# alguoo314/JASPER

Measured on AMD Instinct MI355X. Metric: assembly Mbp/s polished + Gk-mers/s counted, k=37, higher is better.
Workload: dtype u64

## Files before the change

jasper_amd/csrc/polish.hip:

```cpp
#include "polish.hpp"
#include <algorithm>

namespace jk {

constexpr int SMAX = 384;

__device__ __forceinline__ void pyslice(int64_t len, int64_t a, int64_t b, int64_t &lo, int64_t &hi) {
    if (a < 0) { a += len; if (a < 0) a = 0; } else if (a > len) a = len;
    if (b < 0) { b += len; if (b < 0) b = 0; } else if (b > len) b = len;
    if (b < a) b = a;
    lo = a; hi = b;
}

__device__ __forceinline__ int64_t pyround(double x) { return (int64_t)rint(x); }

struct FrontEntry {
    uint32_t node;
    uint16_t tlen;
    uint8_t alive;
    uint8_t pad;
    uint8_t tail[72];
};
static_assert(sizeof(FrontEntry) == 80, "FrontEntry layout");

#ifndef JK_POLISH_TICKS
#define JK_POLISH_TICKS 0
#endif
__device__ __forceinline__ uint64_t phase_clock() { return JK_POLISH_TICKS ? wall_clock64() : 0ull; }

struct Walker {
    TableDev T;
    int k, step, lane;
    uint32_t solid;
    uint8_t *buf;
    int64_t len, gs, glen, cap;
    SegDev *C;
    uint32_t chunk_id;
    uint32_t nrec, naux, seqno, nedit;
    int pass;
    int status;
    uint64_t nlook;
    uint64_t tk[12];
    uint8_t *s_tbf, *s_t1, *s_t2, *s_gkb, *s_gka;
    int64_t delta;
    int64_t dirty_end;
    int64_t glo;
    bool is_first, is_last;
    int spec_fail;
    const uint8_t *cls;
    int64_t cls_n, seg_lo, stop_orig;
    ScratchPool pool;
    uint32_t *bfs_nodes;
    uint8_t *bfs_front, *bfs_patch;
    int bfs_slot;

    __device__ __forceinline__ void guard(int64_t lo, int64_t hi) {
        if ((!is_first && lo < glo) || (!is_last && hi > len)) spec_fail = 1;
    }

    __device__ __forceinline__ uint8_t at(int64_t p) const { return buf[p < gs ? p : p + glen]; }

    struct __attribute__((packed, aligned(1))) U16 { uint32_t w[4]; };

    __device__ __forceinline__ void load_window(int64_t lo, int n, uint32_t w[16]) const {
#pragma unroll
        for (int c = 0; c < 4; ++c) {
            const int64_t s = lo + 16 * c;
            U16 v;
            v.w[0] = v.w[1] = v.w[2] = v.w[3] = 0;
            if (16 * c < n) {
                if (s + 16 <= gs) v = *reinterpret_cast<const U16 *>(buf + s);
                else if (s >= gs && s + glen + 16 <= cap) v = *reinterpret_cast<const U16 *>(buf + s + glen);
                else {
#pragma unroll
                    for (int j = 0; j < 16; ++j) {
                        const int64_t p = s + j;
                        const uint32_t b = p < len ? at(p) : 0u;
                        v.w[j >> 2] |= b << (8 * (j & 3));
                    }
                }
            }
#pragma unroll
            for (int j = 0; j < 4; ++j) w[4 * c + j] = v.w[j];
        }
    }
    __device__ __forceinline__ u128 encode_words(const uint32_t w[16], int lim, int &nvalid) const {
        uint64_t hi = 0, lo = 0, inv = 0;
#pragma unroll
        for (int i = 0; i < 16; ++i) {
            const uint32_t x0 = (w[i] >> 1) & 0x03030303u;
            const uint32_t x = x0 ^ ((x0 >> 1) & 0x01010101u);
            const uint32_t expect = __builtin_amdgcn_perm(0u, 0x54474341u, x);
            const uint32_t d = expect ^ (w[i] & 0xDFDFDFDFu);
            const uint32_t nz = (((d & 0x7F7F7F7Fu) + 0x7F7F7F7Fu) | d) & 0x80808080u;
            const uint32_t c8 = (x * 0x40100401u) >> 24;
            const uint32_t n4 = (((nz >> 7) * 0x01020408u) >> 24) & 0xFu;
            if (i < 8) hi |= (uint64_t)c8 << (56 - 8 * i);
            else lo |= (uint64_t)c8 << (56 - 8 * (i - 8));
            inv |= (uint64_t)n4 << (4 * i);
        }
        if (lim < 64) inv |= ~0ull << lim;
        const int t = inv ? (int)__builtin_ctzll(inv) : 64;
        nvalid = t;
        if (t == 0) return mk(0, 0);
        return shl(shr(mk(hi, lo), 128 - 2 * t), 2 * (k - t));
    }

    __device__ __forceinline__ uint32_t cnt_seq(int64_t a, int64_t b) {
        int64_t lo, hi;
        guard(a, b);
        pyslice(len, a, b, lo, hi);
        const int n = (int)(hi - lo < k ? hi - lo : k);
        uint32_t w[16];
        load_window(lo, n, w);
        int nv;
        const u128 m = encode_words(w, n, nv);
        return clamp32(table_get(T, mix(canonical(m, k), T.B)));
    }
    __device__ __forceinline__ uint32_t cnt_str(const uint8_t *p, int n) const {
        const int lim = n < k ? n : k;
        uint32_t w[16];
#pragma unroll
        for (int x = 0; x < 16; ++x) {
            uint32_t v = 0;
#pragma unroll
            for (int y = 0; y < 4; ++y) {
                const int q = 4 * x + y;
                const uint32_t b = q < lim ? (uint32_t)p[q] : 0u;
                v |= b << (8 * y);
            }
            w[x] = v;
        }
        int nv;
        const u128 m = encode_words(w, lim, nv);
        return clamp32(table_get(T, mix(canonical(m, k), T.B)));
    }

    template <typename F>
    __device__ __forceinline__ uint32_t cnt_fn(int n, F get) const {
        const int lim = n < k ? n : k;
        uint32_t w[16];
#pragma unroll
        for (int x = 0; x < 16; ++x) {
            uint32_t v = 0;
#pragma unroll
            for (int y = 0; y < 4; ++y) {
                const int q = 4 * x + y;
                const uint32_t b = q < lim ? (uint32_t)get(q) : 0u;
                v |= b << (8 * y);
            }
            w[x] = v;
        }
        int nv;
        const u128 m = encode_words(w, lim, nv);
        return clamp32(table_get(T, mix(canonical(m, k), T.B)));
    }

    __device__ void move_gap(int64_t to) {
        if (to == gs) return;
        if (to > gs) {
            const int64_t n = to - gs;
            const uint8_t *src = buf + gs + glen;
            uint8_t *dst = buf + gs;
            int64_t off = 0;
            for (; off + 4096 <= n; off += 4096) {
                U16 v[4];
#pragma unroll
                for (int u = 0; u < 4; ++u) v[u] = *reinterpret_cast<const U16 *>(src + off + (u * 64 + lane) * 16);
#pragma unroll
                for (int u = 0; u < 4; ++u) *reinterpret_cast<U16 *>(dst + off + (u * 64 + lane) * 16) = v[u];
            }
            for (; off < n; off += 256) {
                uint8_t v[4];
#pragma unroll
                for (int u = 0; u < 4; ++u) { int64_t q = off + u * 64 + lane; v[u] = q < n ? src[q] : 0; }
#pragma unroll
                for (int u = 0; u < 4; ++u) { int64_t q = off + u * 64 + lane; if (q < n) dst[q] = v[u]; }
            }
        } else {
            const int64_t n = gs - to;
            const uint8_t *src_end = buf + gs;
            uint8_t *dst_end = buf + gs + glen;
            int64_t off = 0;
            for (; off + 4096 <= n; off += 4096) {
                U16 v[4];
#pragma unroll
                for (int u = 0; u < 4; ++u) v[u] = *reinterpret_cast<const U16 *>(src_end - off - (u * 64 + lane + 1) * 16);
#pragma unroll
                for (int u = 0; u < 4; ++u) *reinterpret_cast<U16 *>(dst_end - off - (u * 64 + lane + 1) * 16) = v[u];
            }
            for (; off < n; off += 256) {
                uint8_t v[4];
#pragma unroll
                for (int u = 0; u < 4; ++u) { int64_t q = off + u * 64 + lane; v[u] = q < n ? src_end[-1 - q] : 0; }
#pragma unroll
                for (int u = 0; u < 4; ++u) { int64_t q = off + u * 64 + lane; if (q < n) dst_end[-1 - q] = v[u]; }
            }
        }
        gs = to;
        __builtin_amdgcn_fence(__ATOMIC_SEQ_CST, "workgroup");
    }
    __device__ void replace(int64_t a, int64_t b, const uint8_t *patch, int64_t plen) {
        const uint64_t tr0 = phase_clock();
        replace_(a, b, patch, plen);
        tk[3] += phase_clock() - tr0;
    }
    __device__ void replace_(int64_t a, int64_t b, const uint8_t *patch, int64_t plen) {
        move_gap(a);
        glen += (b - a);
        if (glen < plen) { status = PS_GAP_EXHAUSTED; return; }
        if (nedit >= C->edit_cap) { status = PS_REC_OVERFLOW; return; }
        if (lane == 0) {
            EditRec e;
            e.a = a; e.plen = (int32_t)plen; e.oldlen = (int32_t)(b - a);
            C->edits[nedit] = e;
        }
        nedit++;
        for (int64_t q = lane; q < plen; q += 64) buf[gs + q] = patch[q];
        gs += plen;
        glen -= plen;
        len += plen - (b - a);
        delta += plen - (b - a);
        dirty_end = a + plen;
        __builtin_amdgcn_fence(__ATOMIC_SEQ_CST, "workgroup");
    }

    __device__ __forceinline__ void cp_seq(uint8_t *dst, int64_t lo, int64_t hi) {
        guard(lo, hi);
        for (int64_t q = lane; q < hi - lo; q += 64) dst[q] = at(lo + q);
    }
    __device__ __forceinline__ void cp_mem(uint8_t *dst, const uint8_t *src, int n) const {
        for (int q = lane; q < n; q += 64) dst[q] = src[q];
    }
    __device__ __forceinline__ void put(uint8_t *dst, uint8_t c) const { if (lane == 0) *dst = c; }
    __device__ __forceinline__ void sync() const { __syncthreads(); }

    __device__ bool check_sequence(const uint8_t *t, int n, uint32_t thr) {
        const int nmid = (n - k > step) ? (n - k - step + step - 1) / step : 0;
        const int jobs = 2 + nmid;
        bool ok = true;
        for (int base = 0; base < jobs; base += 64) {
            const int j = base + lane;
            bool bad = false;
            if (j < jobs) {
                uint32_t c;
                if (j == 0) c = cnt_str(t, n < k ? n : k);
                else if (j == 1) { int lo = n > k ? n - k : 0; c = cnt_str(t + lo, n - lo); }
                else { int i = step * (j - 1); c = cnt_str(t + i, k); }
                bad = c < thr;
            }
            if (__ballot(bad)) ok = false;
        }
        nlook += (uint64_t)jobs;
        return ok;
    }
    __device__ int dense_bad(const uint8_t *t, int n, uint32_t thr) {
        int bad = 0;
        const int nw = n - k + 1;
        for (int base = 0; base < nw; base += 64) {
            const int i = base + lane;
            bool b = false;
            if (i < nw) b = cnt_str(t + i, k) < thr;
            bad += __popcll(__ballot(b));
        }
        if (nw > 0) nlook += (uint64_t)nw;
        return bad;
    }

    __device__ void emit(uint8_t kind, int64_t index, uint8_t newc, uint8_t oldc, uint32_t rep, uint32_t aux_off, uint32_t aux_len) {
        if (nrec >= C->rec_cap) { status = PS_REC_OVERFLOW; return; }
        if (lane == 0) {
            FixRec r;
            r.index = index; r.chunk = chunk_id; r.seqno = seqno; r.pass = (uint8_t)pass; r.kind = kind;
            r.newc = newc; r.oldc = oldc; r.rep = rep; r.aux_off = aux_off; r.aux_len = aux_len;
            C->recs[nrec] = r;
        }
        nrec++;
        seqno++;
    }

    __device__ uint8_t fix_k_case_sub(int L, uint32_t thr, int &outlen) {
        const uint8_t bad = s_tbf[k - 1];
        const char *order = "ACTG";
        for (int b = 0; b < 4; ++b) {
            if ((uint8_t)order[b] == bad) continue;
            cp_mem(s_t1, s_tbf, L);
            sync();
            put(s_t1 + k - 1, (uint8_t)order[b]);
            sync();
            if (check_sequence(s_t1, L, thr)) { outlen = L; return (uint8_t)order[b]; }
            sync();
        }
        return 0;
    }
    __device__ uint8_t fix_insert(int L, uint32_t thr, int &outlen) {
        cp_mem(s_t1, s_tbf, k - 1);
        cp_mem(s_t1 + k - 1, s_tbf + k, L - k);
        sync();
        if (check_sequence(s_t1, L - 1, thr)) { outlen = L - 1; return s_tbf[k - 1]; }
        sync();
        return 0;
    }
    __device__ uint8_t fix_del(int L, uint32_t thr, int &outlen) {
        const char *order = "ATCG";
        for (int a = 0; a < 4; ++a) {
            cp_mem(s_t1, s_tbf, k - 1);
            cp_mem(s_t1 + k, s_tbf + k - 1, L - (k - 1));
            put(s_t1 + k - 1, (uint8_t)order[a]);
            sync();
            if (check_sequence(s_t1, L + 1, thr)) { outlen = L + 1; return (uint8_t)order[a]; }
            sync();
        }
        return 0;
    }
    __device__ uint8_t fixdiploid(int L, uint32_t thr, int64_t gb, int64_t ga, uint8_t &left, uint8_t &right, int &outlen) {
        const uint8_t left_bad = s_tbf[L - k], right_bad = s_tbf[k - 1];
        int64_t gbsi = gb - k + 1; if (gbsi < 0) gbsi = 0;
        const int64_t h = (int64_t)((double)(k - 1 - L + k) / 2.0);
        int64_t alo, ahi, blo, bhi;
        if (ga + k - 1 + h < len) pyslice(len, ga + k - 1, ga + k - 1 + h, alo, ahi);
        else {
            if (!is_last) spec_fail = 1;
            int64_t st = ga + k - 1; if (st > len - 1) st = len - 1; pyslice(len, st, len, alo, ahi);
        }
        const int64_t before_len = ahi - alo;
        int64_t bs = gbsi - before_len + 1; if (bs < 0) bs = 0;
        pyslice(len, bs, gbsi + 1, blo, bhi);
        const int nb = (int)(bhi - blo), na = (int)(ahi - alo);
        if (nb + L + na > SMAX) { status = PS_STRING_TOO_LONG; return 0; }
        const char *order = "ACTG";
        for (int xi = 0; xi < 4; ++xi)
            for (int yi = 0; yi < 4; ++yi) {
                const uint8_t x = (uint8_t)order[xi], y = (uint8_t)order[yi];
                if (x == left_bad && y == right_bad) continue;
                if (x != left_bad && y != right_bad) continue;
                int n = 0;
                int64_t a0, a1;
                pyslice(L, 0, L - k, a0, a1); cp_mem(s_t1 + n, s_tbf + a0, (int)(a1 - a0)); n += (int)(a1 - a0);
                put(s_t1 + n, x); n += 1;
                pyslice(L, L - k + 1, k - 1, a0, a1); cp_mem(s_t1 + n, s_tbf + a0, (int)(a1 - a0)); n += (int)(a1 - a0);
                put(s_t1 + n, y); n += 1;
                pyslice(L, k, L, a0, a1); cp_mem(s_t1 + n, s_tbf + a0, (int)(a1 - a0)); n += (int)(a1 - a0);
                sync();
                cp_seq(s_t2, blo, bhi);
                cp_mem(s_t2 + nb, s_t1, n);
                cp_seq(s_t2 + nb + n, alo, ahi);
                sync();
                const bool ok = check_sequence(s_t2, nb + n + na, thr);
                sync();
                if (ok) { left = x; right = y; outlen = n; return (x == left_bad) ? (uint8_t)'e' : (uint8_t)'s'; }
            }
        return 0;
    }
    __device__ bool fix_same_base_del(int L, uint32_t thr, int &ridx, uint8_t &rbase, int &rrep, int &outlen) {
        if (thr > solid) return false;
        const uint8_t sb = s_tbf[k - 2];
        int inserted = 0;
        const int original_bad = L - k + 1;
        int current_bad = original_bad;
        const int max_ins = original_bad;
        if (L + max_ins > SMAX) { status = PS_STRING_TOO_LONG; return false; }
        while (inserted < max_ins) {
            inserted++;
            const int n = L + inserted;
            cp_mem(s_t1, s_tbf, k - 1);
            for (int q = lane; q < inserted; q += 64) s_t1[k - 1 + q] = sb;
            cp_mem(s_t1 + k - 1 + inserted, s_tbf + k - 1, L - (k - 1));
            sync();
            const int new_bad = dense_bad(s_t1, n, thr);
            sync();
            if (new_bad == 0) { ridx = k - 1; rbase = sb; rrep = inserted; outlen = n; return true; }
            if (new_bad >= current_bad) break;
            current_bad = new_bad;
        }
        const char *order = "ATCG";
        for (int a = 0; a < 4; ++a) {
            cp_mem(s_t1, s_tbf, k - 2);
            put(s_t1 + k - 2, (uint8_t)order[a]);
            cp_mem(s_t1 + k - 1, s_tbf + k - 2, L - (k - 2));
            sync();
            const bool ok = check_sequence(s_t1, L + 1, thr);
            sync();
            if (ok) { ridx = k - 2; rbase = (uint8_t)order[a]; rrep = 1; outlen = L + 1; return true; }
        }
        return false;
    }
    __device__ bool fix_same_base_insertion(int L, uint32_t thr, int &ridx, uint8_t &rbase, int &rrep, int &outlen) {
        if (thr > solid) return false;
        const uint8_t sb = s_tbf[k - 1];
        int deleted = 0;
        const int original_bad = L - k + 1;
        int current_bad = original_bad;
        const int max_del = original_bad;
        while (deleted < max_del) {
            current_bad -= 1;
            deleted += 1;
            const int n = L - deleted;
            if (n < k - 1) break;
            cp_mem(s_t1, s_tbf, k - 1);
            cp_mem(s_t1 + k - 1, s_tbf + k - 1 + deleted, n - (k - 1));
            sync();
            if (n == k) { sync(); break; }
            const int new_bad = dense_bad(s_t1, n, thr);
            sync();
            if (new_bad == 0) { ridx = k - 1; rbase = sb; rrep = deleted; outlen = n; return true; }
            if (new_bad >= current_bad) break;
            current_bad = new_bad;
        }
        {
            const int n1 = L - 1;
            const int nmid = (n1 - k > step) ? (n1 - k - step + step - 1) / step : 0;
            const int jobs = 2 + nmid;
            const int i_first = L - k > 0 ? L - k : 0;
            if (jobs <= 64) {
                const int tpr = 64 / jobs;
                for (int i0 = i_first; i0 < L - 1; i0 += tpr) {
                    const int ti = lane / jobs, j = lane - ti * jobs, i = i0 + ti;
                    const bool active = ti < tpr && i < L - 1;
                    bool bad = false;
                    if (active) {
                        int p, len;
                        if (j == 0) { p = 0; len = n1 < k ? n1 : k; }
                        else if (j == 1) { p = n1 > k ? n1 - k : 0; len = n1 - p; }
                        else { p = step * (j - 1); len = k; }
                        const uint32_t c = cnt_fn(len, [&](int q) { const int sidx = p + q; return s_tbf[sidx < i ? sidx : sidx + 1]; });
                        bad = c < thr;
                    }
                    const uint64_t mb = __ballot(active && bad);
                    for (int tt = 0; tt < tpr && i0 + tt < L - 1; ++tt) {
                        const uint64_t lanes = (jobs == 64 ? ~0ull : ((1ull << jobs) - 1ull)) << (tt * jobs);
                        nlook += (uint64_t)jobs;
                        if ((mb & lanes) == 0ull) {
                            const int iw = i0 + tt;
                            cp_mem(s_t1, s_tbf, iw);
                            cp_mem(s_t1 + iw, s_tbf + iw + 1, L - iw - 1);
                            sync();
                            ridx = iw; rbase = s_tbf[iw]; rrep = 1; outlen = L - 1;
                            return true;
                        }
                    }
                }
                return false;
            }
        }
        for (int i = L - k; i < L - 1; ++i) {
            if (i < 0) continue;
            cp_mem(s_t1, s_tbf, i);
            cp_mem(s_t1 + i, s_tbf + i + 1, L - i - 1);
            sync();
            const bool ok = check_sequence(s_t1, L - 1, thr);
            sync();
            if (ok) { ridx = i; rbase = s_tbf[i]; rrep = 1; outlen = L - 1; return true; }
        }
        return false;
    }

    __device__ int64_t base_extension(int64_t Ltbf, int nb, int na, uint32_t thr) {
        if (nb < k || na < k || thr > solid) return -1;
        uint32_t slot = (uint32_t)((blockIdx.x * 2654435761u) % pool.nslots);
        for (;;) {
            unsigned int old = 1;
            if (lane == 0) old = atomicCAS(&pool.locks[slot], 0u, 1u);
            old = __shfl(old, 0);
            if (old == 0u) break;
            slot = (slot + 1) % pool.nslots;
            __builtin_amdgcn_s_sleep(16);
        }
        bfs_slot = (int)slot;
        __builtin_amdgcn_fence(__ATOMIC_ACQUIRE, "agent");
        uint8_t *sb = pool.base + (size_t)slot * pool.stride;
        bfs_nodes = reinterpret_cast<uint32_t *>(sb);
        bfs_front = sb + pool.off_front;
        bfs_patch = sb + pool.off_patch;
        const int64_t r = base_extension_impl(Ltbf, thr);
        if (r < 0) release_scratch();
        return r;
    }
    __device__ void release_scratch() {
        if (bfs_slot < 0) return;
        __builtin_amdgcn_fence(__ATOMIC_RELEASE, "agent");
        if (lane == 0) atomicExch(&pool.locks[bfs_slot], 0u);
        bfs_slot = -1;
    }
    __device__ int64_t base_extension_impl(int64_t Ltbf, uint32_t thr) {
        const int64_t min_overlap = 5, slack = 10;
        const int64_t max_ext = pyround((double)(Ltbf - 2 * k) * 1.2) + min_overlap + slack;
        const int64_t min_patch_len = pyround((double)(Ltbf - 2 * k) / 1.2) - slack;
        FrontEntry *F = reinterpret_cast<FrontEntry *>(bfs_front);
        const uint32_t fcap = pool.front_cap;
        uint32_t *nodes = bfs_nodes;
        uint32_t nn = 1;
        uint32_t np = 1;
        const int TCAP = k + 3;
        if (lane == 0) {
            nodes[0] = 0;
            F[0].node = 0; F[0].tlen = (uint16_t)k; F[0].alive = 1; F[0].pad = 0;
        }
        for (int q = lane; q < k; q += 64) F[0].tail[q] = s_gkb[q];
        __builtin_amdgcn_fence(__ATOMIC_SEQ_CST, "workgroup");
        const int glo = (k > 5) ? 5 : (k == 5 ? 0 : 5 - k);
        for (int64_t i = 1; i < max_ext; ++i) {
            uint32_t w = 0;
            for (uint32_t base = 0; base < np; base += 64) {
                const uint32_t e = base + lane;
                FrontEntry fe;
                bool alive = false;
                if (e < np) { fe = F[e]; alive = fe.alive != 0; }
                const uint64_t m = __ballot(alive);
                const uint32_t dst = w + (uint32_t)__popcll(m & ((1ull << lane) - 1ull));
                if (alive && dst != e) F[dst] = fe;
                w += (uint32_t)__popcll(m);
            }
            np = w;
            __builtin_amdgcn_fence(__ATOMIC_SEQ_CST, "workgroup");
            if (np > 5000) return -1;
            if (np == 0) return -1;
            const uint32_t last_path = np;
            for (uint32_t g = 0; g < last_path; g += 16) {
                const uint32_t pp = g + (uint32_t)(lane >> 2);
                const int jj = lane & 3;
                uint32_t score = 0;
                if (pp < last_path) {
                    const FrontEntry *fe = &F[pp];
                    const int tl = fe->tlen;
                    const uint8_t bj = (uint8_t)("ACGT"[jj]);
                    uint32_t w[16];
                    const uint8_t *src = fe->tail + (tl - (k - 1));
#pragma unroll
                    for (int c4 = 0; c4 < 4; ++c4) {
                        const U16 v = *reinterpret_cast<const U16 *>(src + 16 * c4);
                        w[4 * c4] = v.w[0]; w[4 * c4 + 1] = v.w[1]; w[4 * c4 + 2] = v.w[2]; w[4 * c4 + 3] = v.w[3];
                    }
                    {
                        const int bi = k - 1;
#pragma unroll
                        for (int x = 0; x < 16; ++x)
                            if (x == (bi >> 2)) w[x] = (w[x] & ~(0xFFu << (8 * (bi & 3)))) | ((uint32_t)bj << (8 * (bi & 3)));
                    }
                    int nv;
                    const u128 m = encode_words(w, k, nv);
                    score = clamp32(table_get(T, mix(canonical(m, k), T.B)));
                }
                const uint32_t gend = (last_path - g) < 16u ? (last_path - g) : 16u;
                nlook += 4ull * gend;
                for (uint32_t q = 0; q < gend; ++q) {
                    const uint32_t p = g + q;
                    int ext = -1;
                    const uint32_t pnode = F[p].node;
                    const int tl = F[p].tlen;
                    for (int j = 0; j < 4; ++j) {
                        const uint32_t sc = __shfl(score, (int)(q * 4 + j));
                        if (sc < thr) continue;
                        const uint8_t bj = (uint8_t)("ACGT"[j]);
                        if (i >= min_overlap && i >= min_patch_len) {
                            struct __attribute__((packed, aligned(1))) U4 { uint32_t v; };
                            const uint32_t last4 = reinterpret_cast<const U4 *>(F[p].tail + (tl - 4))->v;
                            const uint32_t want4 = (uint32_t)s_gka[0] | ((uint32_t)s_gka[1] << 8) | ((uint32_t)s_gka[2] << 16) | ((uint32_t)s_gka[3] << 24);
                            const bool same = last4 == want4 && bj == s_gka[4];
                            if (same) {
                                int n = 0;
                                const int take = tl < TCAP ? tl : TCAP;
                                cp_mem(s_t1, F[p].tail + (tl - take), take); n += take;
                                put(s_t1 + n, bj); n += 1;
                                cp_mem(s_t1 + n, s_gka + glo, k - glo); n += k - glo;
                                sync();
                                const int off = n > 2 * k - 1 ? n - (2 * k - 1) : 0;
                                const bool ok = check_sequence(s_t1 + off, n - off, thr);
                                sync();
                                if (ok) {
                                    if (i == min_overlap) return -1;
                                    const int64_t plen = i - 5;
                                    if (plen > (int64_t)pool.patch_cap) { status = PS_BFS_ARENA; return -1; }
                                    if (lane == 0) {
                                        uint32_t nd = pnode;
                                        for (int u = 0; u < 4; ++u) nd = nodes[nd] >> 2;
                                        for (int64_t u = plen - 1; u >= 0; --u) {
                                            bfs_patch[u] = (uint8_t)("ACGT"[nodes[nd] & 3u]);
                                            nd = nodes[nd] >> 2;
                                        }
                                    }
                                    __builtin_amdgcn_fence(__ATOMIC_SEQ_CST, "workgroup");
                                    return plen;
                                }
                            }
                        }
                        if (ext < 0) {
                            ext = j;
                        } else {
                            if (np >= fcap || nn >= pool.node_cap) { status = PS_BFS_ARENA; return -1; }
                            if (lane == 0) nodes[nn] = (pnode << 2) | (uint32_t)j;
                            const int keep = tl < TCAP ? tl : TCAP - 1;
                            for (int u = lane; u < keep; u += 64) F[np].tail[u] = F[p].tail[tl - keep + u];
                            if (lane == 0) {
                                F[np].tail[keep] = bj;
                                F[np].tlen = (uint16_t)(keep + 1); F[np].node = nn; F[np].alive = 1; F[np].pad = 0;
                            }
                            nn++; np++;
                        }
                    }
                    __builtin_amdgcn_fence(__ATOMIC_SEQ_CST, "workgroup");
                    if (ext >= 0) {
                        if (nn >= pool.node_cap) { status = PS_BFS_ARENA; return -1; }
                        const uint8_t bj = (uint8_t)("ACGT"[ext]);
                        if (lane == 0) nodes[nn] = (pnode << 2) | (uint32_t)ext;
                        if (tl < TCAP) {
                            if (lane == 0) { F[p].tail[tl] = bj; F[p].tlen = (uint16_t)(tl + 1); F[p].node = nn; }
                        } else {
                            uint8_t v = 0;
                            if (lane < TCAP - 1) v = F[p].tail[lane + 1];
                            uint8_t v2 = 0;
                            if (lane + 64 < TCAP - 1) v2 = F[p].tail[lane + 65];
                            __builtin_amdgcn_fence(__ATOMIC_SEQ_CST, "workgroup");
                            if (lane < TCAP - 1) F[p].tail[lane] = v;
                            if (lane + 64 < TCAP - 1) F[p].tail[lane + 64] = v2;
                            if (lane == 0) { F[p].tail[TCAP - 1] = bj; F[p].node = nn; }
                        }
                        nn++;
                    } else if (lane == 0) {
                        F[p].alive = 0;
                    }
                    __builtin_amdgcn_fence(__ATOMIC_SEQ_CST, "workgroup");
                }
            }
        }
        return -1;
    }

    template <typename F>
    __device__ __forceinline__ auto timed(int slot, F f) -> decltype(f()) {
        const uint64_t t0 = phase_clock();
        auto r = f();
        tk[slot] += phase_clock() - t0;
        return r;
    }
    __device__ void fixing_sid(int64_t L64, uint32_t thr, int64_t n, int64_t gb, int64_t ga) {
        int64_t s0 = gb - k + 2; if (s0 < 0) s0 = 0;
        const int L = (int)L64;
        int outlen = 0;
        if (n == k) {
            uint8_t b = timed(4, [&]() { return fix_k_case_sub(L, thr, outlen); });
            if (b) {
                emit('s', ga - 1, b, at(ga - 1), 1, 0, 0);
                replace(s0, ga + k - 1, s_t1, outlen);
            } else {
                b = timed(5, [&]() { return fix_insert(L, thr, outlen); });
                if (b) {
                    emit('i', ga - 1, '-', at(ga - 1), 1, 0, 0);
                    replace(s0, ga + k - 1, s_t1, outlen);
                }
            }
        } else if (n == k - 1) {
            uint8_t b = timed(6, [&]() { return fix_del(L, thr, outlen); });
            if (b) {
                emit('d', ga, b, '-', 1, 0, 0);
                replace(s0, ga + k - 1, s_t1, outlen);
            } else {
                uint8_t left = 0, right = 0;
                const uint8_t lr = timed(7, [&]() { return fixdiploid(L, thr, gb, ga, left, right, outlen); });
                if (lr) {
                    if (lr == 's') emit('s', ga - 1, left, at(ga - 1), 1, 0, 0);
                    else emit('s', gb + 1, right, at(gb + 1), 1, 0, 0);
                    replace(s0, ga + k - 1, s_t1, outlen);
                } else if (status == PS_OK) {
                    int idx = 0, rep = 0; uint8_t bs = 0;
                    if (timed(9, [&]() { return fix_same_base_insertion(L, thr, idx, bs, rep, outlen); })) {
                        emit('i', idx + s0, '-', bs, (uint32_t)rep, 0, 0);
                        replace(s0, ga + k - 1, s_t1, outlen);
                    }
                }
            }
        } else if (n < k - 1 && n > 1 && L64 >= k) {
            int idx = 0, rep = 0; uint8_t bs = 0;
            if (timed(8, [&]() { return fix_same_base_del(L, thr, idx, bs, rep, outlen); })) {
                emit('d', idx + s0, bs, '-', (uint32_t)rep, 0, 0);
                replace(s0, ga + k - 1, s_t1, outlen);
            } else if (status == PS_OK) {
                uint8_t left = 0, right = 0;
                const uint8_t lr = timed(7, [&]() { return fixdiploid(L, thr, gb, ga, left, right, outlen); });
                if (lr) {
                    if (lr == 's') emit('s', ga - 1, left, at(ga - 1), 1, 0, 0);
                    else emit('s', gb + 1, right, at(gb + 1), 1, 0, 0);
                    replace(s0, ga + k - 1, s_t1, outlen);
                } else if (status == PS_OK && timed(9, [&]() { return fix_same_base_insertion(L, thr, idx, bs, rep, outlen); })) {
                    emit('i', idx + s0, '-', bs, (uint32_t)rep, 0, 0);
                    replace(s0, ga + k - 1, s_t1, outlen);
                }
            }
        } else if (n > k) {
            int64_t blo, bhi, alo, ahi;
            guard(gb - k + 1, gb + 1);
            guard(ga, ga + k);
            pyslice(len, gb - k + 1, gb + 1, blo, bhi);
            pyslice(len, ga, ga + k, alo, ahi);
            cp_seq(s_gkb, blo, bhi);
            cp_seq(s_gka, alo, ahi);
            sync();
            const int64_t plen = timed(10, [&]() { return base_extension(L64, (int)(bhi - blo), (int)(ahi - alo), thr); });
            sync();
            if (plen >= 0 && status == PS_OK) {
                int64_t olo, ohi;
                pyslice(len, gb + 1, ga, olo, ohi);
                const int64_t on = ohi - olo;
                if ((uint64_t)naux + (uint64_t)plen + (uint64_t)on > (uint64_t)C->aux_cap) { status = PS_AUX_OVERFLOW; release_scratch(); return; }
                for (int64_t q = lane; q < plen; q += 64) C->aux[naux + q] = bfs_patch[q];
                for (int64_t q = lane; q < on; q += 64) C->aux[naux + plen + q] = at(olo + q);
                emit('x', gb + 1, 0, 0, (uint32_t)on, naux, (uint32_t)plen);
                naux += (uint32_t)(plen + on);
                replace(gb + 1, ga, bfs_patch, plen);
            }
            release_scratch();
        }
    }

    __device__ int64_t handle_bad_kmers(int64_t i, int64_t &wrong, bool fix, int64_t rolling_thre, bool &brk) {
        brk = false;
        const uint64_t th0 = phase_clock();
        uint32_t thre = solid;
        if (rolling_thre > 0) thre = (uint32_t)rolling_thre;
        int64_t j = i - 1;
        for (;;) {
            const int64_t jl = j - lane;
            bool stop = true, oob = false;
            if (!is_first && jl < glo) oob = true;
            else if (jl >= 0) stop = !(cnt_seq(jl, jl + k) < thre);
            const uint64_t m = __ballot(stop);
            nlook += 64;
            if (m) {
                const int f = (int)__builtin_ctzll(m);
                if (__shfl((int)oob, f)) spec_fail = 1;
                j = j - (int64_t)f;
                break;
            }
            j -= 64;
        }
        if (j < -1) j = -1;
        int64_t gb = j + k - 1;
        uint32_t prev = cnt_seq(j, k + j);
        if (j == -1) gb = -1;
        for (;;) {
            const int64_t il = i + lane;
            bool cont = false;
            if (il < len - k + 1) cont = cnt_seq(il, il + k) < thre;
            const bool giveup = cont && rolling_thre != 0 && (il - j > k);
            const uint64_t m = __ballot(!cont || giveup);
            nlook += 64;
            if (m) {
                const int f = (int)__builtin_ctzll(m);
                const bool g = __shfl((int)giveup, f) != 0;
                i += f;
                if (!is_last && i >= len - k + 1) spec_fail = 1;
                if (g) return i + 1;
                break;
            }
            i += 64;
        }
        int64_t ga = i;
        nlook += 4;
        if (2ull * cnt_seq(gb - k + 2, gb + 2) < (uint64_t)solid && 2ull * cnt_seq(gb - k + 3, gb + 3) < (uint64_t)solid) {
        } else if (rolling_thre == 0) {
            while (2ull * cnt_seq(gb - k + 2, gb + 2) >= (uint64_t)prev && gb - k + 1 < ga) {
                if (gb == -1) break;
                if (2ull * prev >= (uint64_t)thre && 2ull * cnt_seq(gb - k + 2, gb + 2) < (uint64_t)thre &&
                    2ull * cnt_seq(gb - k + 3, gb + 3) < (uint64_t)thre) break;
                prev = cnt_seq(gb - k + 2, gb + 2);
                gb++;
                nlook += 4;
            }
            if (gb >= len - 1) { if (!is_last) spec_fail = 1; brk = true; return i; }
        }
        int64_t s0 = gb - k + 2; if (s0 < 0) s0 = 0;
        if (s0 + k + k >= len) { if (!is_last) spec_fail = 1; brk = true; return s0 + k + k; }
        {
            uint32_t c = 0;
            if (lane == 0) c = cnt_seq(s0 + 1, s0 + k + 1);
            else if (lane == 1) c = cnt_seq(s0 + k - 2, s0 + k + k - 2);
            else if (lane == 2) c = cnt_seq(s0 + k - 1, s0 + k + k - 1);
            else if (lane == 3) c = cnt_seq(s0 + k, s0 + k + k);
            const uint64_t lowm = __ballot(lane < 4 && c < thre) & 0xFull;
            nlook += 4;
            if (lowm == 0x7ull) ga = s0 + k;
        }
        int64_t tlo, thi;
        pyslice(len, s0, ga + k - 1, tlo, thi);
        int64_t n = ga - s0; if (n < 0) n = 0;
        wrong += n;
        const uint64_t tf0 = phase_clock();
        tk[1] += tf0 - th0;
        struct FixTimer { uint64_t &acc; uint64_t t0; __device__ ~FixTimer() { acc += phase_clock() - t0; } } fix_timer{tk[2], tf0};
        if (fix) {
            if (gb < 0) return i;
            const int64_t L = thi - tlo;
            if (n <= k) {
                if (L > SMAX) { status = PS_STRING_TOO_LONG; return i; }
                cp_seq(s_tbf, tlo, thi);
                sync();
            }
            fixing_sid(L, thre, n, gb, ga);
            sync();
        }
        return i;
    }

    __device__ int64_t skip_good(int64_t i) {
        const int64_t end = len - k + 1;
        for (;;) {
            const int64_t p = i + (int64_t)lane * (k - 1);
            bool ev = true;
            bool known = false;
            if (p < end && cls != nullptr && p >= dirty_end + k) {
                const int64_t o = p - delta + seg_lo;
                if (!is_last && o >= stop_orig) known = true;
                else if (o >= 0 && o < cls_n) { known = true; ev = cls[o] != PC_CLEAN; }
            }
            if (p < end && !known) {
                uint32_t w[16];
                load_window(p, k, w);
                int nv;
                const u128 m = encode_words(w, k, nv);
                const bool valid = nv == k;
                if (valid) {
                    const uint32_t occ = clamp32(table_get(T, mix(canonical(m, k), T.B)));
                    ev = occ < solid;
                    if (!ev && p > 0) {
                        const int64_t a = p - k > 0 ? p - k : 0;
                        const int64_t b = p > k ? p : k;
                        ev = 50ull * occ < (uint64_t)cnt_seq(a, b);
                    }
                }
            }
            const uint64_t mask = __ballot(ev);
            nlook += 128;
            if (mask) return i + (int64_t)__builtin_ctzll(mask) * (k - 1);
            i += 64ll * (k - 1);
        }
    }

    __device__ void walk(bool fix, int64_t start_i, int64_t &wrong_out, long long &arrive_out) {
        int64_t i = start_i, wrong = 0;
        bool handed_over = false;
        arrive_out = ARRIVE_FAIL;
        while (i < len - k + 1 && status == PS_OK) {
            if (__ballot(spec_fail != 0)) { spec_fail = 1; break; }
            const uint64_t ts0 = phase_clock();
            i = skip_good(i);
            tk[0] += phase_clock() - ts0;
            if (i >= len - k + 1) { if (!is_last) spec_fail = 1; break; }
            if (!is_last && (i - delta + seg_lo) >= stop_orig) {
                if (i < dirty_end + k) spec_fail = 1;
                else { handed_over = true; arrive_out = i - delta + seg_lo; }
                break;
            }
            uint8_t ch = 'A';
            if (lane < k) ch = at(i + lane);
            const uint64_t inwin = (k >= 64) ? ~0ull : ((1ull << k) - 1ull);
            const uint64_t mN = __ballot(ch == 'N') & inwin;
            if (mN) {
                const int f = (int)__builtin_ctzll(mN);
                i += f + 1;
                if (f == 0) {
                    for (;;) {
                        const int64_t q = i + lane;
                        const bool stop = !(q < len - k + 1 && at(q) == 'N');
                        const uint64_t m = __ballot(stop);
                        if (m) { i += (int64_t)__builtin_ctzll(m); break; }
                        i += 64;
                    }
                }
                continue;
            }
            const uint64_t mn = __ballot(ch == 'n') & inwin;
            if (mn) { i += (int64_t)__builtin_ctzll(mn) + 1; continue; }
            const uint64_t mo = __ballot(code(ch) < 0) & inwin;
            if (mo) { i += 1; continue; }
            const uint32_t occ = cnt_seq(i, i + k);
            nlook += 1;
            bool brk = false;
            if (occ < solid) {
                i = handle_bad_kmers(i, wrong, fix, 0, brk);
                if (brk) break;
                continue;
            }
            bool cond2 = false;
            if (i > 0) {
                const int64_t a = i - k > 0 ? i - k : 0;
                const int64_t b = i > k ? i : k;
                cond2 = 50ull * occ < (uint64_t)cnt_seq(a, b);
                nlook += 1;
            }
            if (!cond2) { i += k - 1; continue; }
            int64_t ind0 = i - k > 0 ? i - k : 0;
            int64_t num = (i - ind0 + step - 1) / step;
            double sum = 0.0;
            for (int64_t base = 0; base < num; base += 64) {
                const int64_t t = base + lane;
                unsigned long long c = 0;
                if (t < num) { const int64_t ind = ind0 + (t + 1) * step; c = cnt_seq(ind, ind + k); }
                for (int o = 32; o > 0; o >>= 1) c += __shfl_xor(c, o);
                sum += (double)c;
            }
            nlook += (uint64_t)num;
            const int64_t rolling = pyround(sum / (double)num / 50.0);
            if ((int64_t)occ < rolling) {
                i = handle_bad_kmers(i, wrong, fix, pyround(sum / (double)num / 2.0), brk);
                if (brk) break;
            } else {
                i += k - 1;
            }
        }
        if (!is_last && !handed_over && status == PS_OK) spec_fail = 1;
        if (__ballot(spec_fail != 0)) spec_fail = 1;
        if (is_last && status == PS_OK && !spec_fail) arrive_out = ARRIVE_END;
        if (spec_fail || status != PS_OK) arrive_out = ARRIVE_FAIL;
        wrong_out = wrong;
    }
};

__device__ __forceinline__ void publish_arrival(long long *slot, long long v) {
    if (threadIdx.x == 0) __hip_atomic_store(slot, v, __ATOMIC_RELAXED, __HIP_MEMORY_SCOPE_AGENT);
}

__global__ __launch_bounds__(64, 2) void seg_walk_kernel(TableDev T, SegDev *segs, int n_segs, PolishParams P, int pass, ScratchPool pool,
                                                      unsigned int *ticket) {
    __shared__ uint8_t s_tbf[SMAX], s_t1[SMAX], s_t2[SMAX], s_gkb[64], s_gka[64];
    unsigned int tk = 0;
    if (threadIdx.x == 0) tk = atomicAdd(ticket, 1u);
    const int c = (int)__shfl(tk, 0);
    if (c >= n_segs) return;
    SegDev *C = &segs[c];
    if (C->status != PS_OK) { publish_arrival(C->arrive, ARRIVE_FAIL); return; }
    if (!C->chain_in) publish_arrival(C->arrive, ARRIVE_WALKING);
    const int k = P.k;
    const int lane = threadIdx.x;
    const uint64_t t0 = wall_clock64();
    int64_t start_i = C->start_i;
    if (C->chain_in) {
        const int64_t lo = C->seg_lo + 4ll * k;
        int64_t hi = C->last ? C->cls_n : C->stop_orig + k;
        if (hi > C->cls_n) hi = C->cls_n;
        bool dirty = C->cls == nullptr;
        static_assert(PC_CLEAN == 0, "the clean test below ORs class bytes");
        for (int64_t p0 = lo; p0 < hi && !dirty; p0 += 64 * 16) {
            bool nc = false;
            const int64_t p = p0 + (int64_t)lane * 16;
            if (p + 16 <= hi) {
                struct __attribute__((packed, aligned(1))) V16 { uint32_t w[4]; };
                const V16 v = *reinterpret_cast<const V16 *>(C->cls + p);
                nc = (v.w[0] | v.w[1] | v.w[2] | v.w[3]) != 0u;
            } else {
                for (int q = 0; q < 16; ++q) nc = nc || (p + q < hi && C->cls[p + q] != PC_CLEAN);
            }
            dirty = __ballot(nc) != 0ull;
        }
        if (lane == 0) __hip_atomic_store(C->arrive, dirty ? ARRIVE_WALKING : ARRIVE_CLEAN, __ATOMIC_RELAXED, __HIP_MEMORY_SCOPE_AGENT);
        long long a = ARRIVE_FAIL;
        {
            int back = 1;
            for (uint32_t spins = 0;; ++spins) {
                const int idx = c - back - lane;
                long long v = ARRIVE_FAIL;
                if (idx >= 0) v = __hip_atomic_load(C->arrive - (c - idx), __ATOMIC_RELAXED, __HIP_MEMORY_SCOPE_AGENT);
                const bool published = v >= 0 || v == ARRIVE_FAIL || v == ARRIVE_END;
                const bool skip = v == ARRIVE_CLEAN && !dirty;
                const unsigned long long stopper = __ballot(!skip);
                if (stopper) {
                    const int l = (int)__builtin_ctzll(stopper);
                    const bool ok = (__ballot(published) >> l) & 1ull;
                    if (ok) {
                        a = __shfl(v, l);
                        if (back + l > 1 && a >= 0) {
                            const long long stop = segs[c - 1].stop_orig;
                            if (a < stop) a += ((stop - a + (k - 2)) / (k - 1)) * (long long)(k - 1);
                        }
                        break;
                    }
                    if (spins > (1u << 24)) { a = ARRIVE_FAIL; break; }
                    __builtin_amdgcn_s_sleep(4);
                } else {
                    back += 64;
                    if (spins > (1u << 24)) { a = ARRIVE_FAIL; break; }
                }
            }
        }
        if (a < 0 || a < lo || a - C->seg_lo >= C->len0) {
            if (lane == 0) { C->spec_fail = 1; C->ticks = wall_clock64() - t0; }
            publish_arrival(C->arrive, ARRIVE_FAIL);
            return;
        }
        if (!dirty) {
            const int64_t stop = C->last ? C->cls_n : C->stop_orig;
            const int64_t steps = a >= stop ? 0 : (stop - a + (k - 2)) / (k - 1);
            if (lane == 0) {
                C->took_shortcut = 1;
                C->lookups = 2ull * (uint64_t)steps;
                C->ticks = wall_clock64() - t0;
            }
            publish_arrival(C->arrive, C->last ? ARRIVE_END : a + steps * (k - 1));
            return;
        }
        start_i = a - C->seg_lo;
    }
    Walker w;
    w.T = T; w.k = P.k; w.step = P.step; w.lane = threadIdx.x; w.solid = P.solid;
    w.buf = C->buf; w.len = C->len; w.gs = C->gs; w.glen = C->glen; w.cap = C->cap;
    w.C = C; w.chunk_id = C->chunk; w.nrec = 0; w.naux = 0; w.seqno = 0; w.nedit = 0; w.pass = pass;
    w.status = PS_OK; w.nlook = 0; for (int q = 0; q < 12; ++q) w.tk[q] = 0;
    w.s_tbf = s_tbf; w.s_t1 = s_t1; w.s_t2 = s_t2; w.s_gkb = s_gkb; w.s_gka = s_gka;
    w.delta = 0; w.dirty_end = INT64_MIN / 2; w.glo = P.k;
    w.is_first = C->first != 0; w.is_last = C->last != 0; w.spec_fail = 0;
    w.cls = C->cls; w.cls_n = C->cls_n; w.seg_lo = C->seg_lo; w.stop_orig = C->stop_orig;
    w.pool = pool; w.bfs_slot = -1; w.bfs_nodes = nullptr; w.bfs_front = nullptr; w.bfs_patch = nullptr;
    const bool fix = P.fix && pass < P.passes;
    int64_t wrong = 0;
    long long arrive = ARRIVE_FAIL;
    w.walk(fix, start_i, wrong, arrive);
    w.release_scratch();
    if (threadIdx.x == 0) {
        C->ticks = wall_clock64() - t0;
        for (int q = 0; q < 12; ++q) C->tk[q] = w.tk[q];
        C->len = w.len; C->gs = w.gs; C->glen = w.glen;
        C->nrec = w.nrec; C->naux = w.naux; C->nedit = w.nedit; C->status = w.status; C->spec_fail = w.spec_fail;
        C->wrong = wrong;
        C->lookups = w.nlook;
    }
    publish_arrival(C->arrive, arrive);
}

constexpr int SC_THREADS = 256, SC_GROUP = 16, SC_TILE = SC_THREADS * SC_GROUP, SC_HALO = 4;

__global__ __launch_bounds__(256) void seg_init_kernel(SegDev *segs, int n_segs, const uint8_t *const *chunk_text) {
    struct __attribute__((packed, aligned(1))) V16 { uint32_t w[4]; };
    for (int s = blockIdx.y; s < n_segs; s += gridDim.y) {
        const SegDev S = segs[s];
        const uint8_t *src = chunk_text[S.chunk] + S.seg_lo;
        uint8_t *dst = S.buf + S.glen;
        const int64_t nblk = (S.len0 + 15) >> 4;
        for (int64_t blk = blockIdx.x * (int64_t)blockDim.x + threadIdx.x; blk < nblk; blk += (int64_t)gridDim.x * blockDim.x) {
            const int64_t q0 = blk << 4;
            if (q0 + 16 <= S.len0) *reinterpret_cast<V16 *>(dst + q0) = *reinterpret_cast<const V16 *>(src + q0);
            else for (int64_t q = q0; q < S.len0; ++q) dst[q] = src[q];
        }
    }
}

constexpr uint32_t STITCH_MAX_EDITS = 32;
__global__ __launch_bounds__(256) void seg_stitch_kernel(const SegDev *segs, int n_segs, uint8_t *const *chunk_out, uint8_t *const *cls_out,
                                                         uint8_t *const *flags) {
    struct __attribute__((packed, aligned(1))) V16 { uint32_t w[4]; };
    for (int s = blockIdx.y; s < n_segs; s += gridDim.y) {
        const SegDev S = segs[s];
        uint8_t *dst = chunk_out[S.chunk] + S.out_off;
        uint8_t *cdst = cls_out ? cls_out[S.chunk] + S.out_off : nullptr;
        uint8_t *fl = cls_out ? flags[S.chunk] : nullptr;
        const int64_t n = S.own_hi - S.own_lo;
        const bool all_dirty = S.nedit > STITCH_MAX_EDITS;
        const int64_t nblk = (n + 15) >> 4;
        for (int64_t blk = blockIdx.x * (int64_t)blockDim.x + threadIdx.x; blk < nblk; blk += (int64_t)gridDim.x * blockDim.x) {
            const int64_t q0 = blk << 4;
            const int64_t p0 = S.own_lo + q0;
            const bool full = q0 + 16 <= n;
            bool text_done = false, cls_done = !cdst;
            if (full && (p0 + 16 <= S.gs || p0 >= S.gs)) {
                *reinterpret_cast<V16 *>(dst + q0) = *reinterpret_cast<const V16 *>(S.buf + (p0 < S.gs ? p0 : p0 + S.glen));
                text_done = true;
            }
            if (full && cdst && !all_dirty) {
                int64_t lA = p0, lB = p0 + 15;
                bool uniform = true;
                for (int e = (int)S.nedit - 1; e >= 0; --e) {
                    const EditRec E = S.edits[e];
                    if (lA > E.a + E.plen) { const int64_t d = (int64_t)E.plen - E.oldlen; lA -= d; lB -= d; }
                    else if (lB < E.a - 1) { }
                    else { uniform = false; break; }
                }
                if (uniform && S.seg_lo + lB < S.cls_n) {
                    *reinterpret_cast<V16 *>(cdst + q0) = *reinterpret_cast<const V16 *>(S.cls + S.seg_lo + lA);
                    cls_done = true;
                }
            }
            if (text_done && cls_done) continue;
            const int64_t qe = q0 + 16 < n ? q0 + 16 : n;
            for (int64_t q = q0; q < qe; ++q) {
                const int64_t p = S.own_lo + q;
                if (!text_done) dst[q] = S.buf[p < S.gs ? p : p + S.glen];
                if (cls_done) continue;
                int64_t l = p;
                bool dirty = all_dirty;
                if (!dirty)
                    for (int e = (int)S.nedit - 1; e >= 0; --e) {
                        const EditRec E = S.edits[e];
                        if (l > E.a + E.plen) l -= (int64_t)E.plen - E.oldlen;
                        else if (l >= E.a - 1) { dirty = true; break; }
                    }
                if (dirty) {
                    fl[(S.out_off + q) >> 6] = 1;
                    cdst[q] = PC_OTHER;
                } else {
                    const int64_t old = S.seg_lo + l;
                    cdst[q] = old < S.cls_n ? S.cls[old] : (uint8_t)PC_OTHER;
                }
            }
        }
    }
}

__global__ __launch_bounds__(64) void seg_gather_kernel(const SegDev *segs, int n_segs, const int64_t *idx_base, const uint32_t *seq_base,
                                                        const uint32_t *rec_off, const uint32_t *aux_off, FixRec *out_recs, uint8_t *out_aux) {
    const int s = blockIdx.x;
    if (s >= n_segs) return;
    const SegDev S = segs[s];
    for (uint32_t r = threadIdx.x; r < S.nrec; r += blockDim.x) {
        FixRec f = S.recs[r];
        f.index += idx_base[s];
        f.seqno += seq_base[s];
        if (f.kind == 'x') f.aux_off += aux_off[s];
        out_recs[rec_off[s] + r] = f;
    }
    for (uint32_t q = threadIdx.x; q < S.naux; q += blockDim.x) out_aux[aux_off[s] + q] = S.aux[q];
}

__device__ __forceinline__ long long wave_scan_incl64(long long v) {
    const int lane = threadIdx.x & 63;
#pragma unroll
    for (int o = 1; o < 64; o <<= 1) { const long long u = __shfl_up(v, o); if (lane >= o) v += u; }
    return v;
}
__global__ __launch_bounds__(64) void seg_summary_kernel(SegDev *segs, const int32_t *first_seg, int n_chunks, int64_t *idx_base, uint32_t *seq_base,
                                                         uint32_t *rec_off, uint32_t *aux_off, ChunkSummary *out) {
    const int c = blockIdx.x;
    if (c >= n_chunks) return;
    const int lane = threadIdx.x;
    const int s0 = first_seg[c], s1 = first_seg[c + 1];
    long long newlen = 0, shift = 0, seqc = 0, recc = 0, auxc = 0, wrong = 0, lookups = 0;
    int bad = -1, spec = 0;
    for (int base = s0; base < s1; base += 64) {
        const int s = base + lane;
        const bool in = s < s1;
        long long d = 0, own = 0, nrec = 0, naux = 0, seg_lo = 0, own_hi = 0;
        if (in) {
            SegDev &S = segs[s];
            d = S.len - S.len0;
            own_hi = S.last ? S.len : S.own_hi0 + d;
            own = own_hi - S.own_lo;
            nrec = S.nrec; naux = S.naux; seg_lo = S.seg_lo;
            wrong += S.wrong; lookups += (long long)S.lookups;
            if (S.status != PS_OK && (bad < 0 || s < bad)) bad = s;
            if (S.spec_fail && S.status == PS_OK) spec = 1;
        }
        const long long i_own = wave_scan_incl64(own), i_d = wave_scan_incl64(d), i_rec = wave_scan_incl64(nrec), i_aux = wave_scan_incl64(naux);
        if (in) {
            SegDev &S = segs[s];
            S.own_hi = own_hi;
            S.out_off = newlen + i_own - own;
            idx_base[s] = seg_lo + shift + i_d - d;
            seq_base[s] = (uint32_t)(seqc + i_rec - nrec);
            rec_off[s] = (uint32_t)(recc + i_rec - nrec);
            aux_off[s] = (uint32_t)(auxc + i_aux - naux);
        }
        newlen += __shfl(i_own, 63); shift += __shfl(i_d, 63);
        seqc += __shfl(i_rec, 63); recc += __shfl(i_rec, 63); auxc += __shfl(i_aux, 63);
    }
    for (int o = 32; o > 0; o >>= 1) {
        wrong += __shfl_xor(wrong, o); lookups += __shfl_xor(lookups, o);
        const int b2 = __shfl_xor(bad, o);
        bad = bad < 0 ? b2 : (b2 < 0 ? bad : (b2 < bad ? b2 : bad));
        spec |= __shfl_xor(spec, o);
    }
    if (lane == 0) {
        ChunkSummary R;
        R.newlen = newlen; R.wrong = wrong; R.lookups = (uint64_t)lookups; R.nrec = (uint32_t)recc; R.naux = (uint32_t)auxc; R.bad_seg = bad; R.spec_fail = spec;
        out[c] = R;
    }
}
__global__ __launch_bounds__(64) void seg_offsets_kernel(const int32_t *first_seg, int n_chunks, uint32_t *rec_off, uint32_t *aux_off, const ChunkSummary *sum) {
    const int c = blockIdx.x;
    if (c >= n_chunks || c == 0) return;
    const int lane = threadIdx.x;
    unsigned long long rb = 0, ab = 0;
    for (int q = lane; q < c; q += 64) { rb += sum[q].nrec; ab += sum[q].naux; }
    for (int o = 32; o > 0; o >>= 1) { rb += __shfl_xor(rb, o); ab += __shfl_xor(ab, o); }
    for (int s = first_seg[c] + lane; s < first_seg[c + 1]; s += 64) { rec_off[s] += (uint32_t)rb; aux_off[s] += (uint32_t)ab; }
}

constexpr int SC_BACK = 64;
constexpr int SC_STRIDE = SC_TILE - SC_BACK;
__global__ __launch_bounds__(SC_THREADS) void scan_classify_batch_kernel(const ScanChunk *__restrict__ chunks, int n_chunks, TableDev T, uint32_t solid) {
    __shared__ uint32_t s_code[SC_THREADS + SC_HALO];
    __shared__ uint32_t s_inv[SC_THREADS + SC_HALO];
    __shared__ uint32_t s_cnt[SC_TILE];
    __shared__ uint8_t s_ok[SC_TILE];
    const int t = threadIdx.x;
    const int k = T.k;
    const u128 kmask = maskbits(2 * k);
    for (int ci = blockIdx.y; ci < n_chunks; ci += gridDim.y) {
        const ScanChunk C = chunks[ci];
        const uint8_t *__restrict__ text = C.text;
        const int64_t n = C.len;
        const int64_t nwin = n - k + 1;
        if (nwin <= 0) continue;
        const int64_t ntiles = (n + SC_STRIDE - 1) / SC_STRIDE;
        for (int64_t tile = blockIdx.x; tile < ntiles; tile += gridDim.x) {
            const int64_t origin = tile * SC_STRIDE - SC_BACK;
            uint32_t c, iv;
            stage16(text, origin + (int64_t)t * SC_GROUP, n, c, iv);
            s_code[t + SC_HALO] = c;
            s_inv[t + SC_HALO] = iv;
            if (t < SC_HALO) {
                uint32_t hc, hiv;
                stage16(text, origin - (int64_t)(SC_HALO - t) * SC_GROUP, n, hc, hiv);
                s_code[t] = hc;
                s_inv[t] = hiv;
            }
            __syncthreads();
            const uint32_t w4 = s_code[t], w3 = s_code[t + 1], w2 = s_code[t + 2], w1 = s_code[t + 3];
            const uint64_t ivprev = ((uint64_t)s_inv[t] << 48) | ((uint64_t)s_inv[t + 1] << 32) | ((uint64_t)s_inv[t + 2] << 16) |
                                    (uint64_t)s_inv[t + 3];
            u128 fwd = band(mk(((uint64_t)w4 << 32) | w3, ((uint64_t)w2 << 32) | w1), kmask);
            u128 rc = revcomp(fwd, k);
            int run = ivprev ? (int)__builtin_ctzll(ivprev) : 64;
            const int64_t e0 = origin + (int64_t)t * SC_GROUP;
#pragma unroll
            for (int j0 = 0; j0 < SC_GROUP; j0 += 4) {
                u128 hs[4];
                bool ok[4];
                ulonglong2 ent[4];
#pragma unroll
                for (int u = 0; u < 4; ++u) {
                    const int j = j0 + u;
                    const uint32_t cj = (c >> (30 - 2 * j)) & 3u;
                    const bool bad = (iv >> (15 - j)) & 1u;
                    fwd = band(bor(shl(fwd, 2), mk(0, cj)), kmask);
                    rc = bor(shr(rc, 2), shl(mk(0, 3u - cj), 2 * (k - 1)));
                    run = bad ? 0 : run + 1;
                    const int64_t e = e0 + j;
                    ok[u] = run >= k && e - k + 1 >= 0 && e < n;
                    hs[u] = mix(lt(rc, fwd) ? rc : fwd, T.B);
                    ent[u] = make_ulonglong2(0ull, 0ull);
                    if (ok[u]) ent[u] = *reinterpret_cast<const ulonglong2 *>(read_slots(T, hs[u]) + 2 * home_of(hs[u], T.B, T.s));
                }
#pragma unroll
                for (int u = 0; u < 4; ++u) {
                    s_cnt[t * SC_GROUP + j0 + u] = ok[u] ? clamp32(table_get_prefetched(T, hs[u], ent[u])) : 0u;
                    s_ok[t * SC_GROUP + j0 + u] = ok[u] ? 1 : 0;
                }
            }
            __syncthreads();
            if (t >= SC_BACK / SC_GROUP) {
                struct __attribute__((packed, aligned(1))) V16 { uint32_t w[4]; };
                V16 out;
                out.w[0] = out.w[1] = out.w[2] = out.w[3] = 0;
                const int64_t p0 = e0 - k + 1;
#pragma unroll
                for (int j = 0; j < SC_GROUP; ++j) {
                    const int64_t p = p0 + j;
                    const uint32_t me = s_cnt[t * SC_GROUP + j];
                    uint8_t cl;
                    if (!s_ok[t * SC_GROUP + j]) cl = PC_OTHER;
                    else if (me < solid) cl = PC_BAD;
                    else if (p > 0) {
                        const int64_t qe = (p - k > 0 ? p - k : 0) + k - 1;
                        const int qi = (int)(qe - origin);
                        cl = (!s_ok[qi] || 50ull * me < (unsigned long long)s_cnt[qi]) ? PC_OTHER : PC_CLEAN;
                    } else cl = PC_CLEAN;
                    out.w[j >> 2] |= (uint32_t)cl << (8 * (j & 3));
                }
                if (p0 >= 0 && p0 + SC_GROUP <= nwin) *reinterpret_cast<V16 *>(C.cls + p0) = out;
                else {
#pragma unroll
                    for (int j = 0; j < SC_GROUP; ++j) {
                        const int64_t p = p0 + j;
                        if (p >= 0 && p < nwin) C.cls[p] = (uint8_t)((out.w[j >> 2] >> (8 * (j & 3))) & 0xFFu);
                    }
                }
            }
            __syncthreads();
        }
    }
}

__global__ __launch_bounds__(256) void find_sync_batch_kernel(const ScanChunk *__restrict__ chunks, int n_chunks, int k) {
    struct __attribute__((packed, aligned(1))) V16 { uint32_t w[4]; };
    const int64_t W = 4ll * k;
    for (int ci = blockIdx.y; ci < n_chunks; ci += gridDim.y) {
        const ScanChunk C = chunks[ci];
        if (!C.want_sync) continue;
        const int64_t nwin = C.len - k + 1;
        const uint8_t *__restrict__ cls = C.cls;
        static_assert(PC_CLEAN == 0 && PC_BAD == 1 && PC_OTHER == 2, "the block test below looks at bit 0 of the class bytes");
        const int64_t nblk = (nwin + 15) >> 4;
        for (int64_t blk = blockIdx.x * (int64_t)blockDim.x + threadIdx.x; blk < nblk; blk += (int64_t)gridDim.x * blockDim.x) {
            const int64_t p0 = blk << 4;
            uint32_t w[4];
            if (p0 + 16 <= nwin) {
                const V16 v = *reinterpret_cast<const V16 *>(cls + p0);
                w[0] = v.w[0]; w[1] = v.w[1]; w[2] = v.w[2]; w[3] = v.w[3];
                if (!((w[0] | w[1] | w[2] | w[3]) & 0x01010101u)) continue;
            }
            const int64_t pe = p0 + 16 < nwin ? p0 + 16 : nwin;
            for (int64_t p = p0; p < pe; ++p) {
                if (p < W || p + k - 1 > nwin) continue;
                if (cls[p] != PC_BAD || cls[p - 1] != PC_CLEAN) continue;
                uint32_t diff = 0;
                {
                    int64_t q = p + 1;
                    const int64_t qe = p + k - 1;
                    for (; q + 16 <= qe; q += 16) {
                        const V16 v = *reinterpret_cast<const V16 *>(cls + q);
                        diff |= (v.w[0] ^ 0x01010101u) | (v.w[1] ^ 0x01010101u) | (v.w[2] ^ 0x01010101u) | (v.w[3] ^ 0x01010101u);
                    }
                    for (; q < qe; ++q) diff |= (uint32_t)(cls[q] ^ (uint8_t)PC_BAD);
                    q = p - W;
                    const int64_t qf = p - 1;
                    for (; q + 16 <= qf; q += 16) {
                        const V16 v = *reinterpret_cast<const V16 *>(cls + q);
                        diff |= v.w[0] | v.w[1] | v.w[2] | v.w[3];
                    }
                    for (; q < qf; ++q) diff |= (uint32_t)cls[q];
                }
                if (diff) continue;
                const unsigned int idx = atomicAdd(C.cand_count, 1u);
                if (idx < C.cand_cap) C.cand[idx] = ((int64_t)ci << 40) | p;
            }
        }
    }
}

__global__ __launch_bounds__(256) void rescan_batch_kernel(const ScanChunk *__restrict__ chunks, int n_chunks, TableDev T, uint32_t solid) {
    __shared__ uint32_t s_cnt[4][128];
    __shared__ uint8_t s_valid[4][128];
    __shared__ uint8_t s_text[4][256];
    const int wave = threadIdx.x >> 6, lane = threadIdx.x & 63;
    const int k = T.k;
    for (int ci = blockIdx.y; ci < n_chunks; ci += gridDim.y) {
        const ScanChunk C = chunks[ci];
        const int64_t nwin = C.len - k + 1;
        if (nwin <= 0) continue;
        const int64_t ntile = (nwin + 63) >> 6, nflag = (C.len >> 6) + 1;
        const int64_t W = (int64_t)gridDim.x * 4;
        for (int64_t tile0 = (int64_t)blockIdx.x * 4 + wave; tile0 < ntile; tile0 += 64 * W) {
            uint8_t f = 0;
            {
                const int64_t tl = tile0 + (int64_t)lane * W;
                if (tl < ntile) {
                    f = C.flags[tl];
                    if (tl > 0) f |= C.flags[tl - 1];
                    if (tl + 1 < nflag) f |= C.flags[tl + 1];
                }
            }
            unsigned long long todo = __ballot(f != 0);
          while (todo) {
            const int64_t tile = tile0 + (int64_t)__builtin_ctzll(todo) * W;
            todo &= todo - 1ull;
            const int64_t base = tile * 64 - 64;
#pragma unroll
            for (int q = 0; q < 4; ++q) {
                const int64_t pos = base + (int64_t)lane * 4 + q;
                s_text[wave][lane * 4 + q] = (pos >= 0 && pos < C.len) ? C.text[pos] : (uint8_t)'N';
            }
            __builtin_amdgcn_fence(__ATOMIC_SEQ_CST, "workgroup");
            __builtin_amdgcn_wave_barrier();
#pragma unroll
            for (int r = 0; r < 2; ++r) {
                const int64_t p = base + r * 64 + lane;
                uint32_t cnt = 0;
                uint8_t valid = 0;
                if (p >= 0 && p < nwin) {
                    u128 fwd = mk(0, 0);
                    bool ok = true;
                    for (int j = 0; j < k; ++j) {
                        const int c = code(s_text[wave][r * 64 + lane + j]);
                        ok = ok && c >= 0;
                        fwd = bor(shl(fwd, 2), mk(0, (uint64_t)(c & 3)));
                    }
                    if (ok) {
                        cnt = clamp32(table_get(T, mix(canonical(fwd, k), T.B)));
                        valid = 1;
                    }
                }
                s_cnt[wave][r * 64 + lane] = cnt;
                s_valid[wave][r * 64 + lane] = valid;
            }
            __builtin_amdgcn_fence(__ATOMIC_SEQ_CST, "workgroup");
            __builtin_amdgcn_wave_barrier();
            const int64_t p = tile * 64 + lane;
            if (p < nwin) {
                const int me = 64 + lane;
                uint8_t c;
                if (!s_valid[wave][me]) c = PC_OTHER;
                else if (s_cnt[wave][me] < solid) c = PC_BAD;
                else if (p > 0) {
                    const int qi = p - k > 0 ? me - k : 64;
                    c = (!s_valid[wave][qi] || 50ull * s_cnt[wave][me] < (unsigned long long)s_cnt[wave][qi]) ? PC_OTHER : PC_CLEAN;
                } else c = PC_CLEAN;
                C.cls[p] = c;
            }
            __builtin_amdgcn_wave_barrier();
          }
        }
    }
}

__global__ __launch_bounds__(64) void find_clean_batch_kernel(const ScanChunk *__restrict__ chunks, int n_chunks, int k) {
    const int lane = threadIdx.x;
    for (int ci = blockIdx.y; ci < n_chunks; ci += gridDim.y) {
        const ScanChunk C = chunks[ci];
        const int64_t nwin = C.len - k + 1;
        for (uint32_t g = blockIdx.x; g < C.n_cells; g += gridDim.x) {
            int64_t p0 = (int64_t)g * CLEAN_CELL + CLEAN_CELL / 2;
            const int64_t cell_end = (int64_t)(g + 1) * CLEAN_CELL;
            int64_t cand = -1;
            for (int attempt = 0; attempt < 8; ++attempt) {
                if (p0 - 4ll * k < 0 || p0 + k > nwin || p0 + k > cell_end) break;
                int64_t last_bad = -1;
                for (int64_t q0 = p0 - 4ll * k; q0 < p0 + k; q0 += 64) {
                    const int64_t q = q0 + lane;
                    const bool nc = q < p0 + k && C.cls[q] != PC_CLEAN;
                    const uint64_t m = __ballot(nc);
                    if (m) last_bad = q0 + 63 - (int64_t)__builtin_clzll(m);
                }
                if (last_bad < 0) { cand = p0; break; }
                p0 = last_bad + 4ll * k + 1;
            }
            if (lane == 0) C.clean_cand[g] = cand;
        }
    }
}

static void launch_find_clean(const ScanChunk *d_chunks, int n_chunks, int k, hipStream_t stream) {
    const int gy = n_chunks < 1024 ? n_chunks : 1024;
    const int gx = std::max(1, 8192 / gy);
    hipLaunchKernelGGL(find_clean_batch_kernel, dim3(gx, gy), dim3(64), 0, stream, d_chunks, n_chunks, k);
}

void launch_rescan_batch(const TableDev &T, const ScanChunk *d_chunks, int n_chunks, int k, uint32_t solid, hipStream_t stream) {
    if (n_chunks <= 0) return;
    const int gy = n_chunks < 1024 ? n_chunks : 1024;
    const int gx = std::max(1, 4096 / gy);
    hipLaunchKernelGGL(rescan_batch_kernel, dim3(gx, gy), dim3(256), 0, stream, d_chunks, n_chunks, T, solid);
    hipLaunchKernelGGL(find_sync_batch_kernel, dim3(gx, gy), dim3(256), 0, stream, d_chunks, n_chunks, k);
    launch_find_clean(d_chunks, n_chunks, k, stream);
}

void launch_scan_batch(const TableDev &T, const ScanChunk *d_chunks, int n_chunks, int k, uint32_t solid, hipStream_t stream) {
    if (n_chunks <= 0) return;
    const int gy = n_chunks < 1024 ? n_chunks : 1024;
    const int gx = std::max(1, 4096 / gy);
    hipLaunchKernelGGL(scan_classify_batch_kernel, dim3(gx, gy), dim3(SC_THREADS), 0, stream, d_chunks, n_chunks, T, solid);
    hipLaunchKernelGGL(find_sync_batch_kernel, dim3(gx, gy), dim3(256), 0, stream, d_chunks, n_chunks, k);
    launch_find_clean(d_chunks, n_chunks, k, stream);
}

__global__ __launch_bounds__(256) void copy_chunks_kernel(uint8_t *const *__restrict__ chunk_ptr, uint8_t *__restrict__ pack, const int64_t *__restrict__ offs, int n,
                                                          int to_chunks) {
    for (int c = blockIdx.x; c < n; c += gridDim.x) {
        const int64_t len = offs[c + 1] - offs[c];
        uint8_t *a = chunk_ptr[c], *b = pack + offs[c];
        const uint8_t *src = to_chunks ? b : a;
        uint8_t *dst = to_chunks ? a : b;
        for (int64_t i = threadIdx.x; i < len; i += 256) dst[i] = src[i];
    }
}
void launch_copy_chunks(uint8_t *const *d_chunk_ptr, uint8_t *d_pack, const int64_t *d_offs, int n, bool to_chunks, hipStream_t stream) {
    if (n <= 0) return;
    hipLaunchKernelGGL(copy_chunks_kernel, dim3((unsigned)std::min(n, 256 * 16)), dim3(256), 0, stream, d_chunk_ptr, d_pack, d_offs, n, to_chunks ? 1 : 0);
}

void launch_seg_init(SegDev *d_segs, int n_segs, const uint8_t *const *d_chunk_text, hipStream_t stream) {
    if (n_segs <= 0) return;
    dim3 grid(n_segs >= 512 ? 4 : 64, n_segs < 4096 ? n_segs : 4096);
    hipLaunchKernelGGL(seg_init_kernel, grid, dim3(256), 0, stream, d_segs, n_segs, d_chunk_text);
}
void launch_seg_walk(const TableDev &T, SegDev *d_segs, int n_segs, PolishParams pp, int pass, ScratchPool pool, unsigned int *d_ticket,
                     hipStream_t stream) {
    if (n_segs <= 0) return;
    (void)hipMemsetAsync(d_ticket, 0, sizeof(unsigned int), stream);
    hipLaunchKernelGGL(seg_walk_kernel, dim3(n_segs), dim3(64), 0, stream, T, d_segs, n_segs, pp, pass, pool, d_ticket);
}
void launch_seg_summary(SegDev *d_segs, int n_segs, const int32_t *d_first_seg, int n_chunks, int64_t *idx_base, uint32_t *seq_base, uint32_t *rec_off,
                        uint32_t *aux_off, ChunkSummary *d_out, hipStream_t stream) {
    if (n_segs <= 0 || n_chunks <= 0) return;
    hipLaunchKernelGGL(seg_summary_kernel, dim3(n_chunks), dim3(64), 0, stream, d_segs, d_first_seg, n_chunks, idx_base, seq_base, rec_off, aux_off, d_out);
    hipLaunchKernelGGL(seg_offsets_kernel, dim3(n_chunks), dim3(64), 0, stream, d_first_seg, n_chunks, rec_off, aux_off, d_out);
}
void launch_seg_gather(const SegDev *d_segs, int n_segs, const int64_t *idx_base, const uint32_t *seq_base, const uint32_t *rec_off,
                       const uint32_t *aux_off, FixRec *out_recs, uint8_t *out_aux, hipStream_t stream) {
    if (n_segs <= 0) return;
    hipLaunchKernelGGL(seg_gather_kernel, dim3(n_segs), dim3(64), 0, stream, d_segs, n_segs, idx_base, seq_base, rec_off, aux_off, out_recs, out_aux);
}
void launch_seg_stitch(const SegDev *d_segs, int n_segs, uint8_t *const *d_chunk_out, uint8_t *const *d_cls_out, uint8_t *const *d_flags,
                       hipStream_t stream) {
    if (n_segs <= 0) return;
    dim3 grid(n_segs >= 2048 ? 2 : n_segs >= 512 ? 4 : 64, n_segs < 4096 ? n_segs : 4096);
    hipLaunchKernelGGL(seg_stitch_kernel, grid, dim3(256), 0, stream, d_segs, n_segs, d_chunk_out, d_cls_out, d_flags);
}

}
```

jasper_amd/csrc/polish.hpp:

```cpp
#pragma once
#include "polish_types.hpp"
#include "table.hpp"

namespace jk {

struct ScratchPool {
    unsigned int *locks;
    uint8_t *base;
    size_t stride;
    uint32_t nslots;
    uint32_t node_cap;
    uint32_t front_cap;
    uint32_t patch_cap;
    size_t off_front, off_patch;
};

void launch_scan_batch(const TableDev &T, const ScanChunk *d_chunks, int n_chunks, int k, uint32_t solid, hipStream_t stream);
void launch_rescan_batch(const TableDev &T, const ScanChunk *d_chunks, int n_chunks, int k, uint32_t solid, hipStream_t stream);

void launch_copy_chunks(uint8_t *const *d_chunk_ptr, uint8_t *d_pack, const int64_t *d_offs, int n, bool to_chunks, hipStream_t stream);
void launch_seg_init(SegDev *d_segs, int n_segs, const uint8_t *const *d_chunk_text, hipStream_t stream);
void launch_seg_walk(const TableDev &T, SegDev *d_segs, int n_segs, PolishParams pp, int pass, ScratchPool pool, unsigned int *d_ticket,
                     hipStream_t stream);
void launch_seg_stitch(const SegDev *d_segs, int n_segs, uint8_t *const *d_chunk_out, uint8_t *const *d_cls_out, uint8_t *const *d_flags,
                       hipStream_t stream);
void launch_seg_summary(SegDev *d_segs, int n_segs, const int32_t *d_first_seg, int n_chunks, int64_t *idx_base, uint32_t *seq_base, uint32_t *rec_off,
                        uint32_t *aux_off, ChunkSummary *d_out, hipStream_t stream);
void launch_seg_gather(const SegDev *d_segs, int n_segs, const int64_t *idx_base, const uint32_t *seq_base, const uint32_t *rec_off,
                       const uint32_t *aux_off, FixRec *out_recs, uint8_t *out_aux, hipStream_t stream);

}
```

jasper_amd/csrc/polish_host.hip:

```cpp
#include "polish_host.hpp"
#include <algorithm>
#include <chrono>
#include <cmath>
#include <cstdio>
#include <cstdlib>
#include <cstring>
#include <thread>

namespace jk {

#define HIPCHK(x)                                                                     \
    do {                                                                              \
        hipError_t e_ = (x);                                                          \
        if (e_ != hipSuccess) {                                                       \
            err = std::string(#x) + ": " + hipGetErrorString(e_);                     \
            return -1;                                                                \
        }                                                                             \
    } while (0)
#define STEP(x)                                                                       \
    do {                                                                              \
        if (const int rc_ = (x)) return rc_;                                          \
    } while (0)

namespace {
struct DevBuf {
    void *p = nullptr;
    bool owned = false;
    ~DevBuf() { if (p && owned) (void)hipFree(p); }
    template <typename T> T *as() { return reinterpret_cast<T *>(p); }
};
struct Event {
    hipEvent_t e = nullptr;
    ~Event() { if (e) (void)hipEventDestroy(e); }
};
double now_ms() { return std::chrono::duration<double, std::milli>(std::chrono::steady_clock::now().time_since_epoch()).count(); }

struct LaneOptions {
    bool tight = false;
    std::vector<char> forced;
    bool test_redo_noroom = false;
    int test_nslots = 0;
    bool no_packed_io = false;
    bool host_bookkeeping = false;
    bool debug = false;
    int debug_level = 0;
    void read(int n_chunks, int roomy) {
        tight = !roomy && getenv("JASPER_POLISH_TIGHT") != nullptr;
        forced = parse_forced_redo(getenv("JASPER_POLISH_TEST_REDO"), n_chunks);
        test_redo_noroom = getenv("JASPER_POLISH_TEST_REDO_NOROOM") != nullptr;
        if (const char *e = getenv("JASPER_POLISH_TEST_NSLOTS")) test_nslots = std::max(1, std::min(atoi(e), 256));
        no_packed_io = getenv("JASPER_POLISH_NO_PACKED_IO") != nullptr;
        host_bookkeeping = getenv("JASPER_POLISH_HOST_BOOKKEEPING") != nullptr;
        if (const char *e = getenv("JASPER_POLISH_DEBUG")) { debug = true; debug_level = atoi(e); }
    }
};

struct PolishLane {
    Table &T;
    const int lane;
    hipStream_t st;
    const int n_chunks;
    const char *const *seqs;
    const int64_t *lens;
    const int solid_thre, passes, fix;
    PolishOut &R;
    std::string &err;
    const bool device_in, keep_on_device;
    const int roomy;

    LaneOptions opt;
    LaneLayout L;
    std::vector<int64_t> len;
    std::vector<int> all;
    ScratchPool pool;
    PolishParams pp;
    SegArena arena;
    double t_begin = 0, t_loop = 0;
    Event ev0, ev1;

    int ws_base = 0, pin_base = 0, ws_next = 0;
    DevBuf b_textA, b_textB, b_pack, b_cls, b_clsB, b_flags, b_segedit, b_cells, b_arrive, b_ptrA, b_segs, b_segtext, b_segrec, b_segaux, b_pool, b_locks, b_scan, b_ticket;
    DevBuf b_first, b_sum, b_idx, b_seq, b_ro, b_ao;
    DevBuf b_iooffs;
    static constexpr size_t PIN_RECS = 1u << 18, PIN_AUX = 8u << 20;
    SegDev *segs_p = nullptr;
    int32_t *first_p = nullptr;
    ChunkSummary *sum_p = nullptr;
    int64_t *cand_p = nullptr;
    FixRec *recs_p = nullptr;
    uint8_t *aux_p = nullptr;
    ScanChunk *sc_p = nullptr;
    uint8_t *io_stage = nullptr;
    bool packed_io = false;
    int64_t total_len = 0;
    std::vector<int64_t> io_offs;
    size_t pin_recs_used = 0, pin_aux_used = 0;
    struct PinnedPass { size_t rec_at, nrec, aux_at, naux, r0, pass_i; };
    std::vector<PinnedPass> pinned_passes;

    std::vector<uint8_t *> tables;
    uint8_t **hIn = nullptr, **hOut = nullptr, **hSpare = nullptr;
    uint8_t **dIn = nullptr, **dOut = nullptr, **dSpare = nullptr, **ptrClsIn = nullptr, **ptrClsOut = nullptr, **ptrFlags = nullptr;
    uint8_t *clsIn = nullptr, *clsOut = nullptr;
    int64_t *d_count = nullptr, *d_cells = nullptr, *d_cands = nullptr;

    std::vector<SegDev> segs;
    HostBooks books;
    std::vector<ScanChunk> sc;
    std::vector<int64_t> all_cands;
    std::vector<int64_t> all_cells;
    std::vector<std::vector<int64_t>> chunk_cands;
    std::vector<std::vector<uint8_t>> aux_pass;
    std::vector<size_t> rec_pass_begin;

    int pass = 0;
    size_t ns = 0;
    bool ordinary = true;
    PassCount pc;

    PolishLane(Table &T_, int lane_, hipStream_t st_, int n_chunks_, const char *const *seqs_, const int64_t *lens_, int solid_thre_, int passes_, int fix_,
               PolishOut &R_, std::string &err_, bool device_in_, bool keep_on_device_, int roomy_)
        : T(T_), lane(lane_), st(st_), n_chunks(n_chunks_), seqs(seqs_), lens(lens_), solid_thre(solid_thre_), passes(passes_), fix(fix_), R(R_), err(err_),
          device_in(device_in_), keep_on_device(keep_on_device_), roomy(roomy_) {}

    int run() {
        STEP(setup());
        if (n_chunks == 0) return 0;
        int rc = 0;
        for (int p = 0; p <= passes && rc == 0; ++p) rc = one_pass(p);
        if (opt.debug) { (void)jk_stream_wait(st); fprintf(stderr, "[polish] passes: %.2f ms\n", now_ms() - t_loop); }
        const double t_out = now_ms();
        if (rc == 0) rc = finish();
        (void)jk_stream_wait(st);
        if (opt.debug) fprintf(stderr, "[polish] D2H + record sort: %.2f ms; total %.2f ms\n", now_ms() - t_out, now_ms() - t_begin);
        return rc;
    }

    int one_pass(int p) {
        pass = p;
        STEP(scan());
        STEP(fetch_candidates());
        STEP(cut_and_walk());
        ordinary = !opt.debug && !opt.host_bookkeeping && opt.forced.empty() && summaries_ordinary(sum_p, n_chunks);
        pc.reset(n_chunks);
        if (ordinary) {
            R.n_segments += ns;
            account_summaries(sum_p, n_chunks, pass, passes, pc, R);
        } else {
            STEP(fetch_table());
            STEP(redo());
            if (opt.debug) debug_report();
            ns = segs.size();
            STEP(host_bookkeeping(segs, n_chunks, pass, passes, books, pc, R, err));
        }
        STEP(account_chunks(len.data(), L, pc, pass, passes, R, err));
        STEP(gather());
        return stitch_and_swap();
    }

    bool ws(DevBuf &b, size_t bytes) {
        if (ws_next >= Table::WS_POLISH_MAX) { err = "polish: workspace slots exhausted"; return false; }
        b.p = T.workspace(ws_base + ws_next++, bytes, err);
        b.owned = false;
        return b.p != nullptr;
    }
    template <typename U> U *pin(int slot, size_t bytes) { return reinterpret_cast<U *>(T.pinned(pin_base + slot, bytes, err)); }

    int setup() {
        opt.read(n_chunks, roomy);
        HIPCHK(hipSetDevice(T.device));
        ws_base = lane ? Table::WS_LANE0 + (lane - 1) * Table::WS_POLISH_MAX : 0;
        pin_base = lane * Table::PIN_PER_LANE;
        R.reset(n_chunks);
        if (n_chunks == 0) return 0;
        t_begin = now_ms();
        L = lane_layout(lens, n_chunks, T.k, roomy ? 8 : 1);
        len.assign(lens, lens + n_chunks);
        all.resize(n_chunks);
        for (int c = 0; c < n_chunks; ++c) all[c] = c;
        STEP(allocate());
        STEP(upload());
        if (opt.debug) { (void)jk_stream_wait(st); fprintf(stderr, "[polish] setup + H2D: %.2f ms\n", now_ms() - t_begin); }
        t_loop = now_ms();
        pp.k = L.k;
        pp.step = std::max(2, (int)std::nearbyint((double)L.k / 8.0));
        pp.solid = (uint32_t)solid_thre;
        pp.passes = passes;
        pp.fix = fix ? 1 : 0;
        HIPCHK(hipEventCreate(&ev0.e));
        HIPCHK(hipEventCreate(&ev1.e));
        HIPCHK(hipEventRecord(ev0.e, st));
        return 0;
    }

    int allocate() {
        if (!ws(b_textA, L.text_bytes) || !ws(b_textB, L.text_bytes) ||
            !ws(b_cls, L.pos_items) || !ws(b_clsB, L.pos_items) || !ws(b_flags, L.flag_items) ||
            !ws(b_segedit, L.seg_rec_bound * sizeof(EditRec)) || !ws(b_cells, (2 + L.cell_items + L.cand_items) * 8) ||
            !ws(b_arrive, ((size_t)L.max_segs + 4) * 8) ||
            !ws(b_ptrA, (size_t)6 * n_chunks * sizeof(void *)) ||
            !ws(b_segs, (size_t)L.max_segs * sizeof(SegDev)) || !ws(b_segtext, L.seg_text_bound) ||
            !ws(b_segrec, L.seg_rec_bound * sizeof(FixRec)) || !ws(b_segaux, L.seg_aux_bound))
            return -2;
        pool.nslots = 256;
        pool.node_cap = (uint32_t)(L.RM << 18);
        pool.front_cap = 20480;
        pool.patch_cap = (uint32_t)(L.RM << 16);
        if (roomy) pool.nslots = 64;
        if (opt.test_nslots) pool.nslots = (uint32_t)opt.test_nslots;
        pool.off_front = al256((size_t)pool.node_cap * 4);
        pool.off_patch = pool.off_front + al256((size_t)pool.front_cap * 80);
        pool.stride = pool.off_patch + al256(pool.patch_cap);
        if (!ws(b_pool, pool.stride * pool.nslots) || !ws(b_locks, pool.nslots * 4) || !ws(b_scan, sizeof(ScanChunk) * n_chunks) ||
            !ws(b_ticket, 256)) return -2;
        if (!ws(b_first, ((size_t)n_chunks + 1) * 4) || !ws(b_sum, (size_t)n_chunks * sizeof(ChunkSummary)) || !ws(b_idx, (size_t)L.max_segs * 8) ||
            !ws(b_seq, (size_t)L.max_segs * 4) || !ws(b_ro, (size_t)L.max_segs * 4) || !ws(b_ao, (size_t)L.max_segs * 4)) return -2;
        segs_p = pin<SegDev>(0, (size_t)L.max_segs * sizeof(SegDev));
        first_p = pin<int32_t>(1, ((size_t)n_chunks + 1) * 4);
        sum_p = pin<ChunkSummary>(2, (size_t)n_chunks * sizeof(ChunkSummary));
        cand_p = pin<int64_t>(3, (std::min<size_t>(L.cand_items, 32768) + L.cell_items + 8) * 8);
        recs_p = pin<FixRec>(4, PIN_RECS * sizeof(FixRec));
        aux_p = pin<uint8_t>(5, PIN_AUX);
        sc_p = pin<ScanChunk>(6, sizeof(ScanChunk) * (size_t)n_chunks);
        if (!segs_p || !first_p || !sum_p || !cand_p || !recs_p || !aux_p || !sc_p) return -2;
        for (int c = 0; c < n_chunks; ++c) total_len += len[c];
        packed_io = !device_in && n_chunks > 256 && total_len / n_chunks < 65536 && !opt.no_packed_io;
        if (!packed_io) ws_next += 2;
        if (packed_io) {
            if (!ws(b_iooffs, ((size_t)n_chunks + 1) * 8) || !ws(b_pack, L.text_bytes)) return -2;
            io_offs.resize((size_t)n_chunks + 1);
            io_stage = pin<uint8_t>(7, std::max<size_t>((size_t)total_len, 1) + (size_t)(L.RM * std::max<int64_t>(4096, total_len / 8)) + 64);
            if (!io_stage) return -2;
        }
        pool.base = b_pool.as<uint8_t>();
        pool.locks = b_locks.as<unsigned int>();
        arena.text = b_segtext.as<uint8_t>();
        arena.recs = b_segrec.as<FixRec>();
        arena.edits = b_segedit.as<EditRec>();
        arena.aux = b_segaux.as<uint8_t>();
        arena.arrive = b_arrive.as<long long>();
        arena.text_bound = L.seg_text_bound;
        arena.rec_bound = L.seg_rec_bound;
        arena.aux_bound = L.seg_aux_bound;
        arena.max_segs = L.max_segs;
        d_count = b_cells.as<int64_t>();
        d_cells = d_count + 2;
        d_cands = d_cells + L.cell_items;
        sc.resize(n_chunks);
        all_cands.resize(L.cand_items);
        all_cells.resize(L.cell_items);
        chunk_cands.resize(n_chunks);
        return 0;
    }

    int upload() {
        HIPCHK(hipMemsetAsync(pool.locks, 0, pool.nslots * 4, st));
        clsIn = b_cls.as<uint8_t>();
        clsOut = b_clsB.as<uint8_t>();
        tables.resize((size_t)6 * n_chunks);
        hIn = tables.data();
        hOut = hIn + n_chunks;
        hSpare = hOut + n_chunks;
        uint8_t **hCA = hSpare + n_chunks, **hCB = hCA + n_chunks, **hF = hCB + n_chunks;
        for (int c = 0; c < n_chunks; ++c) {
            uint8_t *a = b_textA.as<uint8_t>() + L.off_text[c];
            hIn[c] = device_in ? reinterpret_cast<uint8_t *>(const_cast<char *>(seqs[c])) : a;
            hOut[c] = b_textB.as<uint8_t>() + L.off_text[c];
            hSpare[c] = a;
            hCA[c] = b_cls.as<uint8_t>() + L.off_pos[c];
            hCB[c] = b_clsB.as<uint8_t>() + L.off_pos[c];
            hF[c] = b_flags.as<uint8_t>() + L.off_flag[c];
            if (len[c] && !device_in && !packed_io) HIPCHK(hipMemcpyAsync(a, seqs[c], (size_t)len[c], hipMemcpyHostToDevice, st));
        }
        HIPCHK(hipMemcpyAsync(b_ptrA.p, tables.data(), tables.size() * sizeof(void *), hipMemcpyHostToDevice, st));
        dIn = b_ptrA.as<uint8_t *>();
        dOut = dIn + n_chunks;
        dSpare = dOut + n_chunks;
        ptrClsIn = dSpare + n_chunks;
        ptrClsOut = ptrClsIn + n_chunks;
        ptrFlags = ptrClsOut + n_chunks;
        if (packed_io) {
            int64_t at = 0;
            for (int c = 0; c < n_chunks; ++c) { io_offs[c] = at; if (len[c]) memcpy(io_stage + at, seqs[c], (size_t)len[c]); at += len[c]; }
            io_offs[n_chunks] = at;
            HIPCHK(hipMemcpyAsync(b_iooffs.p, io_offs.data(), io_offs.size() * 8, hipMemcpyHostToDevice, st));
            if (at) HIPCHK(hipMemcpyAsync(b_pack.p, io_stage, (size_t)at, hipMemcpyHostToDevice, st));
            launch_copy_chunks(dIn, b_pack.as<uint8_t>(), b_iooffs.as<int64_t>(), n_chunks, true, st);
            HIPCHK(hipGetLastError());
            HIPCHK(jk_stream_wait(st));
        }
        return 0;
    }

    int scan() {
        HIPCHK(hipMemsetAsync(d_count, 0, 4, st));
        for (int c = 0; c < n_chunks; ++c) {
            ScanChunk &S = sc[c];
            S.text = hIn[c];
            S.len = len[c];
            S.cls = clsIn + L.off_pos[c];
            S.flags = b_flags.as<uint8_t>() + L.off_flag[c];
            S.cand = d_cands;
            S.cand_count = reinterpret_cast<unsigned int *>(d_count);
            S.cand_cap = (unsigned int)std::min<size_t>(L.cand_items, 0x7fffffffu);
            S.want_sync = want_sync(len[c], L.k, L.geo);
            S.clean_cand = d_cells + L.off_cell[c];
            S.n_cells = scan_cells(L.n_cells[c], len[c], L.k);
        }
        memcpy(sc_p, sc.data(), sizeof(ScanChunk) * n_chunks);
        HIPCHK(hipMemcpyAsync(b_scan.p, sc_p, sizeof(ScanChunk) * n_chunks, hipMemcpyHostToDevice, st));
        if (pass == 0) launch_scan_batch(T.d, b_scan.as<ScanChunk>(), n_chunks, L.k, pp.solid, st);
        else launch_rescan_batch(T.d, b_scan.as<ScanChunk>(), n_chunks, L.k, pp.solid, st);
        HIPCHK(hipGetLastError());
        return 0;
    }

    int fetch_candidates() {
        const size_t CAND_PRE = std::min<size_t>(L.cand_items, 32768);
        HIPCHK(hipMemcpyAsync(cand_p, d_count, (2 + L.cell_items + CAND_PRE) * 8, hipMemcpyDeviceToHost, st));
        HIPCHK(jk_stream_wait(st));
        unsigned int n_cand = *reinterpret_cast<const unsigned int *>(cand_p);
        if (L.cell_items) memcpy(all_cells.data(), cand_p + 2, L.cell_items * 8);
        if (CAND_PRE) memcpy(all_cands.data(), cand_p + 2 + L.cell_items, std::min<size_t>(n_cand, CAND_PRE) * 8);
        n_cand = (unsigned int)std::min<size_t>(n_cand, L.cand_items);
        if (n_cand > CAND_PRE) {
            HIPCHK(hipMemcpyAsync(all_cands.data() + CAND_PRE, d_cands + CAND_PRE, (n_cand - CAND_PRE) * 8, hipMemcpyDeviceToHost, st));
            HIPCHK(jk_stream_wait(st));
        }
        group_candidates(all_cands.data(), n_cand, n_chunks, chunk_cands);
        return 0;
    }

    CutInput cut_input() const { return CutInput{len.data(), &chunk_cands, all_cells.data(), clsIn, opt.tight}; }

    int cut_and_walk() {
        const double tb0 = opt.debug ? now_ms() : 0;
        arena.rewind();
        STEP(build_segment_table(L, cut_input(), all, true, arena, segs_p, ns, first_p, err));
        const double tb1 = opt.debug ? now_ms() : 0;
        STEP(run_segments(segs_p, ns, true));
        if (opt.debug) fprintf(stderr, "[polish]   host: build %zu segments %.3f ms, upload + walk + summary %.3f ms\n", ns, tb1 - tb0, now_ms() - tb1);
        return 0;
    }

    int run_segments(SegDev *sv, size_t nsv, bool summary) {
        if (!nsv) return 0;
        const bool fine = opt.debug && opt.debug_level >= 2;
        double tf[5] = {fine ? now_ms() : 0, 0, 0, 0, 0};
        if (hipMemcpyAsync(b_segs.p, sv, nsv * sizeof(SegDev), hipMemcpyHostToDevice, st) != hipSuccess) { err = "polish: H2D segs"; return -1; }
        if (summary && hipMemcpyAsync(b_first.p, first_p, ((size_t)n_chunks + 1) * 4, hipMemcpyHostToDevice, st) != hipSuccess) { err = "polish: H2D first"; return -1; }
        if (fine) { (void)jk_stream_wait(st); tf[1] = now_ms(); }
        launch_seg_init(b_segs.as<SegDev>(), (int)nsv, (const uint8_t *const *)dIn, st);
        if (hipMemsetAsync(b_arrive.p, 0x80, (nsv + 2) * 8, st) != hipSuccess) { err = "polish: memset"; return -1; }
        if (fine) { (void)jk_stream_wait(st); tf[2] = now_ms(); }
        launch_seg_walk(T.d, b_segs.as<SegDev>(), (int)nsv, pp, pass, pool, b_ticket.as<unsigned int>(), st);
        if (hipGetLastError() != hipSuccess) { err = "polish: kernel launch failed"; return -1; }
        if (fine) { (void)jk_stream_wait(st); tf[3] = now_ms(); }
        if (summary) {
            launch_seg_summary(b_segs.as<SegDev>(), (int)nsv, b_first.as<int32_t>(), n_chunks, b_idx.as<int64_t>(), b_seq.as<uint32_t>(), b_ro.as<uint32_t>(),
                               b_ao.as<uint32_t>(), b_sum.as<ChunkSummary>(), st);
            if (hipMemcpyAsync(sum_p, b_sum.p, (size_t)n_chunks * sizeof(ChunkSummary), hipMemcpyDeviceToHost, st) != hipSuccess) { err = "polish: D2H summary"; return -1; }
        } else if (hipMemcpyAsync(sv, b_segs.p, nsv * sizeof(SegDev), hipMemcpyDeviceToHost, st) != hipSuccess) { err = "polish: D2H segs"; return -1; }
        if (jk_stream_wait(st) != hipSuccess) { err = "polish: kernel execution failed"; return -1; }
        if (fine) {
            tf[4] = now_ms();
            fprintf(stderr, "[polish]     %zu segments x %zu B: H2D %.3f ms, init + memset %.3f ms, walk %.3f ms, %s %.3f ms\n", nsv, sizeof(SegDev), tf[1] - tf[0], tf[2] - tf[1],
                    tf[3] - tf[2], summary ? "summary + D2H" : "D2H", tf[4] - tf[3]);
        }
        return 0;
    }

    int fetch_table() {
        segs.resize(ns);
        HIPCHK(hipMemcpyAsync(segs.data(), b_segs.p, ns * sizeof(SegDev), hipMemcpyDeviceToHost, st));
        HIPCHK(jk_stream_wait(st));
        R.n_segments += segs.size();
        return 0;
    }

    int redo() {
        std::vector<char> failed;
        const std::vector<int> again = chunks_to_redo(segs, opt.forced, n_chunks, failed);
        if (again.empty()) return 0;
        R.n_respeculated += again.size();
        std::vector<SegDev> redo_segs((size_t)L.max_segs);
        size_t nredo = 0;
        SegArena behind = arena;
        std::string no_room;
        const bool fits = build_segment_table(L, cut_input(), again, false, behind, redo_segs.data(), nredo, nullptr, no_room) == 0;
        if (opt.test_redo_noroom || !fits) {
            segs.assign((size_t)L.max_segs, SegDev{});
            size_t nall = 0;
            arena.rewind();
            STEP(build_segment_table(L, cut_input(), all, false, arena, segs.data(), nall, nullptr, err));
            segs.resize(nall);
            return run_segments(segs.data(), segs.size(), false);
        }
        redo_segs.resize(nredo);
        STEP(run_segments(redo_segs.data(), redo_segs.size(), false));
        merge_redo(segs, failed, redo_segs);
        return 0;
    }

    void debug_report() const {
        uint64_t mx = 0, sum = 0, mxl = 0; int64_t mxlen = 0; size_t nrecs = 0, mxrec = 0;
        uint64_t tks[12] = {0, 0, 0, 0, 0, 0, 0, 0, 0, 0, 0, 0}, mxtk[12] = {0, 0, 0, 0, 0, 0, 0, 0, 0, 0, 0, 0};
        for (const SegDev &S : segs) {
            sum += S.ticks; nrecs += S.nrec;
            for (int q = 0; q < 12; ++q) tks[q] += S.tk[q];
            if (S.ticks > mx) { mx = S.ticks; mxl = S.lookups; mxlen = S.len0; mxrec = S.nrec; for (int q = 0; q < 12; ++q) mxtk[q] = S.tk[q]; }
        }
        fprintf(stderr, "[polish] pass %d: %zu segments, %zu records, walk ticks(10ns): mean %.0f max %llu (that segment: len %lld, %llu lookups, %zu records)\n",
                pass, segs.size(), nrecs, segs.empty() ? 0.0 : (double)sum / segs.size(), (unsigned long long)mx, (long long)mxlen,
                (unsigned long long)mxl, mxrec);
        fprintf(stderr, "[polish]   of all walk ticks: skip_good %.1f%%, find run %.1f%%, choose fix %.1f%% (of which splice %.1f%%)\n",
                100.0 * tks[0] / (sum + 1), 100.0 * tks[1] / (sum + 1), 100.0 * tks[2] / (sum + 1), 100.0 * tks[3] / (sum + 1));
        fprintf(stderr, "[polish]   inside choose fix: k_case_sub %.1f%%, insert %.1f%%, del %.1f%%, diploid %.1f%%, same_base_del %.1f%%, same_base_ins %.1f%%, path search %.1f%%\n",
                100.0 * tks[4] / (sum + 1), 100.0 * tks[5] / (sum + 1), 100.0 * tks[6] / (sum + 1), 100.0 * tks[7] / (sum + 1),
                100.0 * tks[8] / (sum + 1), 100.0 * tks[9] / (sum + 1), 100.0 * tks[10] / (sum + 1));
        fprintf(stderr, "[polish]   slowest segment (10ns ticks): skip %llu, find run %llu, choose fix %llu [sub %llu ins %llu del %llu diploid %llu sb_del %llu sb_ins %llu path %llu], splice %llu\n",
                (unsigned long long)mxtk[0], (unsigned long long)mxtk[1], (unsigned long long)mxtk[2], (unsigned long long)mxtk[4], (unsigned long long)mxtk[5],
                (unsigned long long)mxtk[6], (unsigned long long)mxtk[7], (unsigned long long)mxtk[8], (unsigned long long)mxtk[9], (unsigned long long)mxtk[10],
                (unsigned long long)mxtk[3]);
        int hb[8] = {0, 0, 0, 0, 0, 0, 0, 0};
        for (const SegDev &S : segs) { double ms = S.ticks * 1e-5; int b = ms < 0.1 ? 0 : ms < 0.3 ? 1 : ms < 1 ? 2 : ms < 2 ? 3 : ms < 4 ? 4 : ms < 8 ? 5 : ms < 16 ? 6 : 7; hb[b]++; }
        fprintf(stderr, "[polish]   segments by walk time: <0.1ms %d, <0.3 %d, <1 %d, <2 %d, <4 %d, <8 %d, <16 %d, more %d\n", hb[0], hb[1], hb[2], hb[3], hb[4], hb[5], hb[6], hb[7]);
    }

    int gather() {
        rec_pass_begin.push_back(R.recs.size());
        aux_pass.emplace_back();
        if (!ordinary) {
            HIPCHK(hipMemcpyAsync(b_segs.p, segs.data(), ns * sizeof(SegDev), hipMemcpyHostToDevice, st));
            HIPCHK(hipMemcpyAsync(b_idx.p, books.idx_base.data(), ns * 8, hipMemcpyHostToDevice, st));
            HIPCHK(hipMemcpyAsync(b_seq.p, books.seq_base.data(), ns * 4, hipMemcpyHostToDevice, st));
            HIPCHK(hipMemcpyAsync(b_ro.p, books.rec_off.data(), ns * 4, hipMemcpyHostToDevice, st));
            HIPCHK(hipMemcpyAsync(b_ao.p, books.aux_off.data(), ns * 4, hipMemcpyHostToDevice, st));
        }
        if (!pc.nrec) return 0;
        DevBuf d_recs, d_aux;
        const int ws_save = ws_next;
        if (!ws(d_recs, pc.nrec * sizeof(FixRec)) || !ws(d_aux, pc.naux)) return -2;
        ws_next = ws_save;
        launch_seg_gather(b_segs.as<SegDev>(), (int)ns, b_idx.as<int64_t>(), b_seq.as<uint32_t>(), b_ro.as<uint32_t>(), b_ao.as<uint32_t>(), d_recs.as<FixRec>(),
                          d_aux.as<uint8_t>(), st);
        HIPCHK(hipGetLastError());
        const size_t r0 = R.recs.size();
        R.recs.resize(r0 + pc.nrec);
        aux_pass.back().resize(pc.naux);
        if (pin_recs_used + pc.nrec <= PIN_RECS && pin_aux_used + pc.naux <= PIN_AUX) {
            HIPCHK(hipMemcpyAsync(recs_p + pin_recs_used, d_recs.p, pc.nrec * sizeof(FixRec), hipMemcpyDeviceToHost, st));
            if (pc.naux) HIPCHK(hipMemcpyAsync(aux_p + pin_aux_used, d_aux.p, pc.naux, hipMemcpyDeviceToHost, st));
            pinned_passes.push_back(PinnedPass{pin_recs_used, pc.nrec, pin_aux_used, pc.naux, r0, aux_pass.size() - 1});
            pin_recs_used += pc.nrec;
            pin_aux_used += pc.naux;
        } else {
            HIPCHK(hipMemcpyAsync(&R.recs[r0], d_recs.p, pc.nrec * sizeof(FixRec), hipMemcpyDeviceToHost, st));
            if (pc.naux) HIPCHK(hipMemcpyAsync(aux_pass.back().data(), d_aux.p, pc.naux, hipMemcpyDeviceToHost, st));
            HIPCHK(jk_stream_wait(st));
        }
        return 0;
    }

    int stitch_and_swap() {
        const bool carry = pass < passes;
        if (carry) HIPCHK(hipMemsetAsync(b_flags.p, 0, L.flag_items, st));
        launch_seg_stitch(b_segs.as<SegDev>(), (int)ns, (uint8_t *const *)dOut, carry ? (uint8_t *const *)ptrClsOut : nullptr,
                          carry ? (uint8_t *const *)ptrFlags : nullptr, st);
        HIPCHK(hipGetLastError());
        for (int c = 0; c < n_chunks; ++c) len[c] = pc.newlen[c];
        if (!ordinary) HIPCHK(jk_stream_wait(st));
        std::swap(hIn, hOut);
        std::swap(dIn, dOut);
        if (pass == 0) { hOut = hSpare; dOut = dSpare; }
        std::swap(clsIn, clsOut);
        std::swap(ptrClsIn, ptrClsOut);
        return 0;
    }

    int finish() {
        HIPCHK(hipEventRecord(ev1.e, st));
        if (keep_on_device) {
            R.d_seqs.resize(n_chunks);
            R.d_lens.assign(len.begin(), len.end());
            for (int c = 0; c < n_chunks; ++c) R.d_seqs[c] = hIn[c];
        }
        bool packed_back = false;
        if (packed_io && !keep_on_device) {
            int64_t at = 0;
            for (int c = 0; c < n_chunks; ++c) { io_offs[c] = at; at += len[c]; }
            io_offs[n_chunks] = at;
            if ((size_t)at <= L.text_bytes && (size_t)at <= (size_t)total_len + (size_t)(L.RM * std::max<int64_t>(4096, total_len / 8)) + 64) {
                packed_back = true;
                HIPCHK(hipMemcpyAsync(b_iooffs.p, io_offs.data(), io_offs.size() * 8, hipMemcpyHostToDevice, st));
                launch_copy_chunks(dIn, b_pack.as<uint8_t>(), b_iooffs.as<int64_t>(), n_chunks, false, st);
                HIPCHK(hipGetLastError());
                if (at) HIPCHK(hipMemcpyAsync(io_stage, b_pack.p, (size_t)at, hipMemcpyDeviceToHost, st));
            }
        }
        for (int c = 0; c < n_chunks && !keep_on_device && !packed_back; ++c) {
            R.seqs[c].resize((size_t)len[c]);
            if (len[c]) HIPCHK(hipMemcpyAsync(&R.seqs[c][0], hIn[c], (size_t)len[c], hipMemcpyDeviceToHost, st));
        }
        HIPCHK(jk_stream_wait(st));
        if (packed_back)
            for (int c = 0; c < n_chunks; ++c) R.seqs[c].assign(reinterpret_cast<const char *>(io_stage) + io_offs[c], (size_t)len[c]);
        float ms = 0;
        HIPCHK(hipEventElapsedTime(&ms, ev0.e, ev1.e));
        R.seconds = ms * 1e-3;
        for (const PinnedPass &P : pinned_passes) {
            memcpy(&R.recs[P.r0], recs_p + P.rec_at, P.nrec * sizeof(FixRec));
            if (P.naux) memcpy(aux_pass[P.pass_i].data(), aux_p + P.aux_at, P.naux);
        }
        regroup_and_sort(R, rec_pass_begin, aux_pass);
        return 0;
    }
};
}

int run_polish(Table &T, int n_chunks, const char *const *seqs, const int64_t *lens, int solid_thre, int passes, int fix,
               PolishOut &R, std::string &err, bool device_in, bool keep_on_device, int roomy) {
    HIPCHK(hipSetDevice(T.device));
    if (T.materialize(err)) return -1;
    int lanes = T.polish_calls++ >= 1 && n_chunks >= 12 ? 3 : 1;
    if (const char *e = getenv("JASPER_POLISH_LANES")) lanes = atoi(e);
    if (getenv("JASPER_POLISH_DEBUG")) lanes = 1;
    lanes = std::max(1, std::min(std::min(lanes, (int)Table::POLISH_LANES_MAX), n_chunks / 2));
    if (lanes == 1) return PolishLane(T, 0, T.stream, n_chunks, seqs, lens, solid_thre, passes, fix, R, err, device_in, keep_on_device, roomy).run();

    std::vector<int> order(n_chunks);
    for (int c = 0; c < n_chunks; ++c) order[c] = c;
    std::stable_sort(order.begin(), order.end(), [&](int a, int b) { return lens[a] > lens[b]; });
    std::vector<std::vector<int>> mine(lanes);
    std::vector<int64_t> load(lanes, 0);
    for (int c : order) {
        int l = 0;
        for (int j = 1; j < lanes; ++j) if (load[j] < load[l]) l = j;
        mine[l].push_back(c);
        load[l] += lens[c];
    }
    for (auto &m : mine) std::sort(m.begin(), m.end());
    if (!T.polish_ev) HIPCHK(hipEventCreateWithFlags(&T.polish_ev, hipEventDisableTiming));
    HIPCHK(hipEventRecord(T.polish_ev, T.stream));
    for (int l = 1; l < lanes; ++l) {
        if (!T.polish_stream[l]) HIPCHK(hipStreamCreateWithFlags(&T.polish_stream[l], hipStreamNonBlocking));
        HIPCHK(hipStreamWaitEvent(T.polish_stream[l], T.polish_ev, 0));
    }
    std::vector<PolishOut> out(lanes);
    std::vector<std::string> errs(lanes);
    std::vector<int> rcs(lanes, 0);
    std::vector<std::vector<const char *>> lseqs(lanes);
    std::vector<std::vector<int64_t>> llens(lanes);
    for (int l = 0; l < lanes; ++l)
        for (int c : mine[l]) { lseqs[l].push_back(seqs[c]); llens[l].push_back(lens[c]); }
    auto run = [&](int l) {
        rcs[l] = PolishLane(T, l, l ? T.polish_stream[l] : T.stream, (int)mine[l].size(), lseqs[l].data(), llens[l].data(), solid_thre, passes, fix, out[l], errs[l],
                            device_in, keep_on_device, roomy).run();
    };
    {
        std::vector<std::thread> th;
        for (int l = 1; l < lanes; ++l) th.emplace_back(run, l);
        run(0);
        for (auto &t : th) t.join();
    }
    for (int want : {-1, -4, -2})
        for (int l = 0; l < lanes; ++l)
            if (rcs[l] == want) { err = errs[l]; return want; }
    for (int l = 0; l < lanes; ++l)
        if (rcs[l]) { err = errs[l]; return rcs[l]; }
    R.reset(n_chunks);
    if (keep_on_device) { R.d_seqs.assign(n_chunks, nullptr); R.d_lens.assign(n_chunks, 0); }
    for (int l = 0; l < lanes; ++l) {
        PolishOut &O = out[l];
        for (size_t j = 0; j < mine[l].size(); ++j) {
            const int c = mine[l][j];
            R.seqs[c].swap(O.seqs[j]);
            R.aux[c].swap(O.aux[j]);
            if (keep_on_device) { R.d_seqs[c] = O.d_seqs[j]; R.d_lens[c] = O.d_lens[j]; }
            for (int q = 0; q < 4; ++q) R.qv_chunk[4 * (size_t)c + q] = O.qv_chunk[4 * j + q];
        }
        for (FixRec f : O.recs) { f.chunk = (uint32_t)mine[l][f.chunk]; R.recs.push_back(f); }
        for (int q = 0; q < 4; ++q) R.qv[q] += O.qv[q];
        R.lookups += O.lookups;
        R.n_segments += O.n_segments;
        R.n_respeculated += O.n_respeculated;
        R.seconds = std::max(R.seconds, O.seconds);
    }
    sort_records(R.recs);
    return 0;
}

}
```

Baseline: 3068.

## Fuse polish pass kernels and memsets into piece-based init/finish launches

Merges the stitch, gather and offset kernels into one seg_finish kernel that splits segments into fixed-size pieces for load balance. The arrive/flag/ticket memsets move into seg_init. find_sync and find_clean are fused into one launch. Records and aux are copied back in a single D2H transfer. This cuts launch and memset overhead and evens out work across long and short segments, at the cost of more complex indexing and host-side piece construction.

```diff
diff --git a/jasper_amd/csrc/polish.hip b/jasper_amd/csrc/polish.hip
--- a/jasper_amd/csrc/polish.hip
+++ b/jasper_amd/csrc/polish.hip
@@ -1027,95 +1027,135 @@
 
 constexpr int SC_THREADS = 256, SC_GROUP = 16, SC_TILE = SC_THREADS * SC_GROUP, SC_HALO = 4;
 
-__global__ __launch_bounds__(256) void seg_init_kernel(SegDev *segs, int n_segs, const uint8_t *const *chunk_text) {
+__device__ __forceinline__ void piece_range(const SegPiece P, int64_t n, int64_t &q_lo, int64_t &q_hi) {
+    q_lo = (int64_t)(P.piece & ~SEG_PIECE_LAST) * SEG_PIECE;
+    q_hi = (P.piece & SEG_PIECE_LAST) ? n : q_lo + SEG_PIECE;
+    if (q_hi > n) q_hi = n;
+}
+
+__global__ __launch_bounds__(256) void seg_init_kernel(const SegDev *__restrict__ segs, const SegPiece *__restrict__ work, int n_work,
+                                                       const uint8_t *const *__restrict__ chunk_text, PassPreset Z) {
     struct __attribute__((packed, aligned(1))) V16 { uint32_t w[4]; };
-    for (int s = blockIdx.y; s < n_segs; s += gridDim.y) {
-        const SegDev S = segs[s];
-        const uint8_t *src = chunk_text[S.chunk] + S.seg_lo;
-        uint8_t *dst = S.buf + S.glen;
-        const int64_t nblk = (S.len0 + 15) >> 4;
-        for (int64_t blk = blockIdx.x * (int64_t)blockDim.x + threadIdx.x; blk < nblk; blk += (int64_t)gridDim.x * blockDim.x) {
-            const int64_t q0 = blk << 4;
-            if (q0 + 16 <= S.len0) *reinterpret_cast<V16 *>(dst + q0) = *reinterpret_cast<const V16 *>(src + q0);
-            else for (int64_t q = q0; q < S.len0; ++q) dst[q] = src[q];
+    const int64_t gt = (int64_t)blockIdx.x * blockDim.x + threadIdx.x, gn = (int64_t)gridDim.x * blockDim.x;
+    for (int64_t i = gt; i < Z.n_arrive; i += gn) Z.arrive[i] = ARRIVE_PENDING;
+    for (int64_t i = gt; i < Z.n_flag16; i += gn) reinterpret_cast<uint4 *>(Z.flags)[i] = make_uint4(0u, 0u, 0u, 0u);
+    if (gt == 0) {
+        *Z.ticket = 0u;
+        if (Z.cand_count) *Z.cand_count = 0u;
+    }
+    for (int w = blockIdx.x; w < n_work; w += gridDim.x) {
+        const SegPiece P = work[w];
+        const SegDev *__restrict__ S = segs + P.seg;
+        const int64_t len0 = S->len0;
+        const uint8_t *src = chunk_text[S->chunk] + S->seg_lo;
+        uint8_t *dst = S->buf + S->glen;
+        int64_t q_lo, q_hi;
+        piece_range(P, len0, q_lo, q_hi);
+        for (int64_t q0 = q_lo + (int64_t)threadIdx.x * 16; q0 < q_hi; q0 += (int64_t)blockDim.x * 16) {
+            if (q0 + 16 <= len0) *reinterpret_cast<V16 *>(dst + q0) = *reinterpret_cast<const V16 *>(src + q0);
+            else for (int64_t q = q0; q < len0; ++q) dst[q] = src[q];
         }
     }
 }
 
 constexpr uint32_t STITCH_MAX_EDITS = 32;
-__global__ __launch_bounds__(256) void seg_stitch_kernel(const SegDev *segs, int n_segs, uint8_t *const *chunk_out, uint8_t *const *cls_out,
-                                                         uint8_t *const *flags) {
+__global__ __launch_bounds__(256) void seg_finish_kernel(const SegDev *__restrict__ segs, int n_segs, const SegPiece *__restrict__ work, int n_work,
+                                                         uint8_t *const *__restrict__ chunk_out, uint8_t *const *__restrict__ cls_out,
+                                                         uint8_t *const *__restrict__ flags, const int64_t *__restrict__ idx_base,
+                                                         const uint32_t *__restrict__ seq_base, const uint32_t *__restrict__ rec_off,
+                                                         const uint32_t *__restrict__ aux_off, const ChunkSummary *__restrict__ sum, FixRec *out_recs,
+                                                         uint8_t *out_aux) {
     struct __attribute__((packed, aligned(1))) V16 { uint32_t w[4]; };
-    for (int s = blockIdx.y; s < n_segs; s += gridDim.y) {
-        const SegDev S = segs[s];
-        uint8_t *dst = chunk_out[S.chunk] + S.out_off;
-        uint8_t *cdst = cls_out ? cls_out[S.chunk] + S.out_off : nullptr;
-        uint8_t *fl = cls_out ? flags[S.chunk] : nullptr;
-        const int64_t n = S.own_hi - S.own_lo;
-        const bool all_dirty = S.nedit > STITCH_MAX_EDITS;
-        const int64_t nblk = (n + 15) >> 4;
-        for (int64_t blk = blockIdx.x * (int64_t)blockDim.x + threadIdx.x; blk < nblk; blk += (int64_t)gridDim.x * blockDim.x) {
-            const int64_t q0 = blk << 4;
-            const int64_t p0 = S.own_lo + q0;
-            const bool full = q0 + 16 <= n;
-            bool text_done = false, cls_done = !cdst;
-            if (full && (p0 + 16 <= S.gs || p0 >= S.gs)) {
-                *reinterpret_cast<V16 *>(dst + q0) = *reinterpret_cast<const V16 *>(S.buf + (p0 < S.gs ? p0 : p0 + S.glen));
-                text_done = true;
-            }
-            if (full && cdst && !all_dirty) {
-                int64_t lA = p0, lB = p0 + 15;
-                bool uniform = true;
-                for (int e = (int)S.nedit - 1; e >= 0; --e) {
-                    const EditRec E = S.edits[e];
-                    if (lA > E.a + E.plen) { const int64_t d = (int64_t)E.plen - E.oldlen; lA -= d; lB -= d; }
-                    else if (lB < E.a - 1) { }
-                    else { uniform = false; break; }
-                }
-                if (uniform && S.seg_lo + lB < S.cls_n) {
-                    *reinterpret_cast<V16 *>(cdst + q0) = *reinterpret_cast<const V16 *>(S.cls + S.seg_lo + lA);
-                    cls_done = true;
-                }
-            }
-            if (text_done && cls_done) continue;
-            const int64_t qe = q0 + 16 < n ? q0 + 16 : n;
-            for (int64_t q = q0; q < qe; ++q) {
-                const int64_t p = S.own_lo + q;
-                if (!text_done) dst[q] = S.buf[p < S.gs ? p : p + S.glen];
-                if (cls_done) continue;
-                int64_t l = p;
-                bool dirty = all_dirty;
-                if (!dirty)
-                    for (int e = (int)S.nedit - 1; e >= 0; --e) {
-                        const EditRec E = S.edits[e];
-                        if (l > E.a + E.plen) l -= (int64_t)E.plen - E.oldlen;
-                        else if (l >= E.a - 1) { dirty = true; break; }
-                    }
-                if (dirty) {
-                    fl[(S.out_off + q) >> 6] = 1;
-                    cdst[q] = PC_OTHER;
-                } else {
-                    const int64_t old = S.seg_lo + l;
-                    cdst[q] = old < S.cls_n ? S.cls[old] : (uint8_t)PC_OTHER;
-                }
-            }
-        }
-    }
-}
-
-__global__ __launch_bounds__(64) void seg_gather_kernel(const SegDev *segs, int n_segs, const int64_t *idx_base, const uint32_t *seq_base,
-                                                        const uint32_t *rec_off, const uint32_t *aux_off, FixRec *out_recs, uint8_t *out_aux) {
-    const int s = blockIdx.x;
-    if (s >= n_segs) return;
-    const SegDev S = segs[s];
-    for (uint32_t r = threadIdx.x; r < S.nrec; r += blockDim.x) {
-        FixRec f = S.recs[r];
-        f.index += idx_base[s];
-        f.seqno += seq_base[s];
-        if (f.kind == 'x') f.aux_off += aux_off[s];
-        out_recs[rec_off[s] + r] = f;
-    }
-    for (uint32_t q = threadIdx.x; q < S.naux; q += blockDim.x) out_aux[aux_off[s] + q] = S.aux[q];
+    __shared__ EditRec s_edits[STITCH_MAX_EDITS];
+    if ((int)blockIdx.x >= n_work) {
+        const int lane = threadIdx.x & 63;
+        const int s = ((int)blockIdx.x - n_work) * 4 + (threadIdx.x >> 6);
+        if (s >= n_segs) return;
+        const SegDev *__restrict__ S = segs + s;
+        const uint32_t nrec = S->nrec, naux = S->naux;
+        if (!(nrec | naux)) return;
+        uint32_t rb = rec_off[s], ab = aux_off[s];
+        if (sum) {
+            const int c = (int)S->chunk;
+            uint32_t r = 0, a = 0;
+            for (int q = lane; q < c; q += 64) { r += sum[q].nrec; a += sum[q].naux; }
+            for (int o = 32; o > 0; o >>= 1) { r += __shfl_xor(r, o); a += __shfl_xor(a, o); }
+            rb += r; ab += a;
+        }
+        const FixRec *recs = S->recs;
+        const uint8_t *aux = S->aux;
+        const int64_t ib = idx_base[s];
+        const uint32_t sb = seq_base[s];
+        for (uint32_t r = lane; r < nrec; r += 64) {
+            FixRec f = recs[r];
+            f.index += ib;
+            f.seqno += sb;
+            if (f.kind == 'x') f.aux_off += ab;
+            out_recs[rb + r] = f;
+        }
+        for (uint32_t q = lane; q < naux; q += 64) out_aux[ab + q] = aux[q];
+        return;
+    }
+    const SegPiece P = work[blockIdx.x];
+    const SegDev *__restrict__ S = segs + P.seg;
+    const uint32_t chunk = S->chunk, nedit = S->nedit;
+    const int64_t own_lo = S->own_lo, out_off = S->out_off, gs = S->gs, glen = S->glen, seg_lo = S->seg_lo, cls_n = S->cls_n;
+    const int64_t n = S->own_hi - own_lo;
+    const uint8_t *buf = S->buf, *cls = S->cls;
+    uint8_t *dst = chunk_out[chunk] + out_off;
+    uint8_t *cdst = cls_out ? cls_out[chunk] + out_off : nullptr;
+    uint8_t *fl = cls_out ? flags[chunk] : nullptr;
+    const bool all_dirty = nedit > STITCH_MAX_EDITS;
+    const int ne = (cdst && !all_dirty) ? (int)nedit : 0;
+    if ((int)threadIdx.x < ne) s_edits[threadIdx.x] = S->edits[threadIdx.x];
+    __syncthreads();
+    int64_t q_lo, q_hi;
+    piece_range(P, n, q_lo, q_hi);
+    for (int64_t q0 = q_lo + (int64_t)threadIdx.x * 16; q0 < q_hi; q0 += (int64_t)blockDim.x * 16) {
+        const int64_t p0 = own_lo + q0;
+        const bool full = q0 + 16 <= n;
+        bool text_done = false, cls_done = !cdst;
+        if (full && (p0 + 16 <= gs || p0 >= gs)) {
+            *reinterpret_cast<V16 *>(dst + q0) = *reinterpret_cast<const V16 *>(buf + (p0 < gs ? p0 : p0 + glen));
+            text_done = true;
+        }
+        if (full && cdst && !all_dirty) {
+            int64_t lA = p0, lB = p0 + 15;
+            bool uniform = true;
+            for (int e = ne - 1; e >= 0; --e) {
+                const EditRec E = s_edits[e];
+                if (lA > E.a + E.plen) { const int64_t d = (int64_t)E.plen - E.oldlen; lA -= d; lB -= d; }
+                else if (lB < E.a - 1) { }
+                else { uniform = false; break; }
+            }
+            if (uniform && seg_lo + lB < cls_n) {
+                *reinterpret_cast<V16 *>(cdst + q0) = *reinterpret_cast<const V16 *>(cls + seg_lo + lA);
+                cls_done = true;
+            }
+        }
+        if (text_done && cls_done) continue;
+        const int64_t qe = q0 + 16 < n ? q0 + 16 : n;
+        for (int64_t q = q0; q < qe; ++q) {
+            const int64_t p = own_lo + q;
+            if (!text_done) dst[q] = buf[p < gs ? p : p + glen];
+            if (cls_done) continue;
+            int64_t l = p;
+            bool dirty = all_dirty;
+            if (!dirty)
+                for (int e = ne - 1; e >= 0; --e) {
+                    const EditRec E = s_edits[e];
+                    if (l > E.a + E.plen) l -= (int64_t)E.plen - E.oldlen;
+                    else if (l >= E.a - 1) { dirty = true; break; }
+                }
+            if (dirty) {
+                fl[(out_off + q) >> 6] = 1;
+                cdst[q] = PC_OTHER;
+            } else {
+                const int64_t old = seg_lo + l;
+                cdst[q] = old < cls_n ? cls[old] : (uint8_t)PC_OTHER;
+            }
+        }
+    }
 }
 
 __device__ __forceinline__ long long wave_scan_incl64(long long v) {
@@ -1171,16 +1211,6 @@
         out[c] = R;
     }
 }
-__global__ __launch_bounds__(64) void seg_offsets_kernel(const int32_t *first_seg, int n_chunks, uint32_t *rec_off, uint32_t *aux_off, const ChunkSummary *sum) {
-    const int c = blockIdx.x;
-    if (c >= n_chunks || c == 0) return;
-    const int lane = threadIdx.x;
-    unsigned long long rb = 0, ab = 0;
-    for (int q = lane; q < c; q += 64) { rb += sum[q].nrec; ab += sum[q].naux; }
-    for (int o = 32; o > 0; o >>= 1) { rb += __shfl_xor(rb, o); ab += __shfl_xor(ab, o); }
-    for (int s = first_seg[c] + lane; s < first_seg[c + 1]; s += 64) { rec_off[s] += (uint32_t)rb; aux_off[s] += (uint32_t)ab; }
-}
-
 constexpr int SC_BACK = 64;
 constexpr int SC_STRIDE = SC_TILE - SC_BACK;
 __global__ __launch_bounds__(SC_THREADS) void scan_classify_batch_kernel(const ScanChunk *__restrict__ chunks, int n_chunks, TableDev T, uint32_t solid) {
@@ -1277,7 +1307,7 @@
     }
 }
 
-__global__ __launch_bounds__(256) void find_sync_batch_kernel(const ScanChunk *__restrict__ chunks, int n_chunks, int k) {
+__device__ __forceinline__ void find_sync_blocks(const ScanChunk *__restrict__ chunks, int n_chunks, int k, int bx, int gx) {
     struct __attribute__((packed, aligned(1))) V16 { uint32_t w[4]; };
     const int64_t W = 4ll * k;
     for (int ci = blockIdx.y; ci < n_chunks; ci += gridDim.y) {
@@ -1287,7 +1317,7 @@
         const uint8_t *__restrict__ cls = C.cls;
         static_assert(PC_CLEAN == 0 && PC_BAD == 1 && PC_OTHER == 2, "the block test below looks at bit 0 of the class bytes");
         const int64_t nblk = (nwin + 15) >> 4;
-        for (int64_t blk = blockIdx.x * (int64_t)blockDim.x + threadIdx.x; blk < nblk; blk += (int64_t)gridDim.x * blockDim.x) {
+        for (int64_t blk = bx * (int64_t)blockDim.x + threadIdx.x; blk < nblk; blk += (int64_t)gx * blockDim.x) {
             const int64_t p0 = blk << 4;
             uint32_t w[4];
             if (p0 + 16 <= nwin) {
@@ -1399,12 +1429,12 @@
     }
 }
 
-__global__ __launch_bounds__(64) void find_clean_batch_kernel(const ScanChunk *__restrict__ chunks, int n_chunks, int k) {
-    const int lane = threadIdx.x;
+__device__ __forceinline__ void find_clean_waves(const ScanChunk *__restrict__ chunks, int n_chunks, int k, int wx, int gw) {
+    const int lane = threadIdx.x & 63;
     for (int ci = blockIdx.y; ci < n_chunks; ci += gridDim.y) {
         const ScanChunk C = chunks[ci];
         const int64_t nwin = C.len - k + 1;
-        for (uint32_t g = blockIdx.x; g < C.n_cells; g += gridDim.x) {
+        for (uint32_t g = (uint32_t)wx; g < C.n_cells; g += (uint32_t)gw) {
             int64_t p0 = (int64_t)g * CLEAN_CELL + CLEAN_CELL / 2;
             const int64_t cell_end = (int64_t)(g + 1) * CLEAN_CELL;
             int64_t cand = -1;
@@ -1425,10 +1455,14 @@
     }
 }
 
-static void launch_find_clean(const ScanChunk *d_chunks, int n_chunks, int k, hipStream_t stream) {
-    const int gy = n_chunks < 1024 ? n_chunks : 1024;
-    const int gx = std::max(1, 8192 / gy);
-    hipLaunchKernelGGL(find_clean_batch_kernel, dim3(gx, gy), dim3(64), 0, stream, d_chunks, n_chunks, k);
+__global__ __launch_bounds__(256) void find_cuts_batch_kernel(const ScanChunk *__restrict__ chunks, int n_chunks, int k, int sync_gx) {
+    if ((int)blockIdx.x < sync_gx) find_sync_blocks(chunks, n_chunks, k, (int)blockIdx.x, sync_gx);
+    else find_clean_waves(chunks, n_chunks, k, ((int)blockIdx.x - sync_gx) * 4 + (int)(threadIdx.x >> 6), ((int)gridDim.x - sync_gx) * 4);
+}
+
+static void launch_find_cuts(const ScanChunk *d_chunks, int n_chunks, int k, int gx, int gy, hipStream_t stream) {
+    const int clean_gx = (std::max(1, 8192 / gy) + 3) / 4;
+    hipLaunchKernelGGL(find_cuts_batch_kernel, dim3(gx + clean_gx, gy), dim3(256), 0, stream, d_chunks, n_chunks, k, gx);
 }
 
 void launch_rescan_batch(const TableDev &T, const ScanChunk *d_chunks, int n_chunks, int k, uint32_t solid, hipStream_t stream) {
@@ -1436,8 +1470,7 @@
     const int gy = n_chunks < 1024 ? n_chunks : 1024;
     const int gx = std::max(1, 4096 / gy);
     hipLaunchKernelGGL(rescan_batch_kernel, dim3(gx, gy), dim3(256), 0, stream, d_chunks, n_chunks, T, solid);
-    hipLaunchKernelGGL(find_sync_batch_kernel, dim3(gx, gy), dim3(256), 0, stream, d_chunks, n_chunks, k);
-    launch_find_clean(d_chunks, n_chunks, k, stream);
+    launch_find_cuts(d_chunks, n_chunks, k, gx, gy, stream);
 }
 
 void launch_scan_batch(const TableDev &T, const ScanChunk *d_chunks, int n_chunks, int k, uint32_t solid, hipStream_t stream) {
@@ -1445,8 +1478,7 @@
     const int gy = n_chunks < 1024 ? n_chunks : 1024;
     const int gx = std::max(1, 4096 / gy);
     hipLaunchKernelGGL(scan_classify_batch_kernel, dim3(gx, gy), dim3(SC_THREADS), 0, stream, d_chunks, n_chunks, T, solid);
-    hipLaunchKernelGGL(find_sync_batch_kernel, dim3(gx, gy), dim3(256), 0, stream, d_chunks, n_chunks, k);
-    launch_find_clean(d_chunks, n_chunks, k, stream);
+    launch_find_cuts(d_chunks, n_chunks, k, gx, gy, stream);
 }
 
 __global__ __launch_bounds__(256) void copy_chunks_kernel(uint8_t *const *__restrict__ chunk_ptr, uint8_t *__restrict__ pack, const int64_t *__restrict__ offs, int n,
@@ -1464,33 +1496,28 @@
     hipLaunchKernelGGL(copy_chunks_kernel, dim3((unsigned)std::min(n, 256 * 16)), dim3(256), 0, stream, d_chunk_ptr, d_pack, d_offs, n, to_chunks ? 1 : 0);
 }
 
-void launch_seg_init(SegDev *d_segs, int n_segs, const uint8_t *const *d_chunk_text, hipStream_t stream) {
-    if (n_segs <= 0) return;
-    dim3 grid(n_segs >= 512 ? 4 : 64, n_segs < 4096 ? n_segs : 4096);
-    hipLaunchKernelGGL(seg_init_kernel, grid, dim3(256), 0, stream, d_segs, n_segs, d_chunk_text);
+void launch_seg_init(const SegDev *d_segs, const SegPiece *d_work, int n_work, const uint8_t *const *d_chunk_text, const PassPreset &preset,
+                     hipStream_t stream) {
+    if (n_work <= 0) return;
+    hipLaunchKernelGGL(seg_init_kernel, dim3(n_work), dim3(256), 0, stream, d_segs, d_work, n_work, d_chunk_text, preset);
 }
 void launch_seg_walk(const TableDev &T, SegDev *d_segs, int n_segs, PolishParams pp, int pass, ScratchPool pool, unsigned int *d_ticket,
                      hipStream_t stream) {
     if (n_segs <= 0) return;
-    (void)hipMemsetAsync(d_ticket, 0, sizeof(unsigned int), stream);
     hipLaunchKernelGGL(seg_walk_kernel, dim3(n_segs), dim3(64), 0, stream, T, d_segs, n_segs, pp, pass, pool, d_ticket);
 }
 void launch_seg_summary(SegDev *d_segs, int n_segs, const int32_t *d_first_seg, int n_chunks, int64_t *idx_base, uint32_t *seq_base, uint32_t *rec_off,
                         uint32_t *aux_off, ChunkSummary *d_out, hipStream_t stream) {
     if (n_segs <= 0 || n_chunks <= 0) return;
     hipLaunchKernelGGL(seg_summary_kernel, dim3(n_chunks), dim3(64), 0, stream, d_segs, d_first_seg, n_chunks, idx_base, seq_base, rec_off, aux_off, d_out);
-    hipLaunchKernelGGL(seg_offsets_kernel, dim3(n_chunks), dim3(64), 0, stream, d_first_seg, n_chunks, rec_off, aux_off, d_out);
-}
-void launch_seg_gather(const SegDev *d_segs, int n_segs, const int64_t *idx_base, const uint32_t *seq_base, const uint32_t *rec_off,
-                       const uint32_t *aux_off, FixRec *out_recs, uint8_t *out_aux, hipStream_t stream) {
-    if (n_segs <= 0) return;
-    hipLaunchKernelGGL(seg_gather_kernel, dim3(n_segs), dim3(64), 0, stream, d_segs, n_segs, idx_base, seq_base, rec_off, aux_off, out_recs, out_aux);
-}
-void launch_seg_stitch(const SegDev *d_segs, int n_segs, uint8_t *const *d_chunk_out, uint8_t *const *d_cls_out, uint8_t *const *d_flags,
-                       hipStream_t stream) {
-    if (n_segs <= 0) return;
-    dim3 grid(n_segs >= 2048 ? 2 : n_segs >= 512 ? 4 : 64, n_segs < 4096 ? n_segs : 4096);
-    hipLaunchKernelGGL(seg_stitch_kernel, grid, dim3(256), 0, stream, d_segs, n_segs, d_chunk_out, d_cls_out, d_flags);
-}
-
-}
+}
+void launch_seg_finish(const SegDev *d_segs, int n_segs, const SegPiece *d_work, int n_work, uint8_t *const *d_chunk_out, uint8_t *const *d_cls_out,
+                       uint8_t *const *d_flags, const int64_t *idx_base, const uint32_t *seq_base, const uint32_t *rec_off, const uint32_t *aux_off,
+                       const ChunkSummary *d_sum, FixRec *out_recs, uint8_t *out_aux, hipStream_t stream) {
+    if (n_segs <= 0 || n_work <= 0) return;
+    const int gather_blocks = out_recs ? (n_segs + 3) / 4 : 0;
+    hipLaunchKernelGGL(seg_finish_kernel, dim3(n_work + gather_blocks), dim3(256), 0, stream, d_segs, n_segs, d_work, n_work, d_chunk_out, d_cls_out, d_flags,
+                       idx_base, seq_base, rec_off, aux_off, d_sum, out_recs, out_aux);
+}
+
+}
diff --git a/jasper_amd/csrc/polish.hpp b/jasper_amd/csrc/polish.hpp
--- a/jasper_amd/csrc/polish.hpp
+++ b/jasper_amd/csrc/polish.hpp
@@ -19,14 +19,39 @@
 void launch_rescan_batch(const TableDev &T, const ScanChunk *d_chunks, int n_chunks, int k, uint32_t solid, hipStream_t stream);
 
 void launch_copy_chunks(uint8_t *const *d_chunk_ptr, uint8_t *d_pack, const int64_t *d_offs, int n, bool to_chunks, hipStream_t stream);
-void launch_seg_init(SegDev *d_segs, int n_segs, const uint8_t *const *d_chunk_text, hipStream_t stream);
+constexpr int64_t SEG_PIECE = 4096;
+constexpr uint32_t SEG_PIECE_LAST = 0x80000000u;
+struct SegPiece {
+    uint32_t seg;
+    uint32_t piece;
+};
+inline size_t make_pieces(const SegDev *segs, size_t n_segs, SegPiece *out) {
+    size_t n = 0;
+    for (size_t s = 0; s < n_segs; ++s) {
+        const int64_t own = (segs[s].last ? segs[s].len0 : segs[s].own_hi0) - segs[s].own_lo;
+        const uint32_t np = own > SEG_PIECE ? (uint32_t)((own + SEG_PIECE - 1) / SEG_PIECE) : 1u;
+        for (uint32_t p = 0; p < np; ++p) out[n++] = SegPiece{(uint32_t)s, p + 1 == np ? (p | SEG_PIECE_LAST) : p};
+    }
+    return n;
+}
+inline size_t max_pieces(size_t max_segs, size_t text_bytes) { return max_segs + text_bytes / (size_t)SEG_PIECE + 1; }
+
+struct PassPreset {
+    long long *arrive;
+    int64_t n_arrive;
+    unsigned int *ticket;
+    unsigned int *cand_count;
+    uint8_t *flags;
+    int64_t n_flag16;
+};
+void launch_seg_init(const SegDev *d_segs, const SegPiece *d_work, int n_work, const uint8_t *const *d_chunk_text, const PassPreset &preset,
+                     hipStream_t stream);
 void launch_seg_walk(const TableDev &T, SegDev *d_segs, int n_segs, PolishParams pp, int pass, ScratchPool pool, unsigned int *d_ticket,
                      hipStream_t stream);
-void launch_seg_stitch(const SegDev *d_segs, int n_segs, uint8_t *const *d_chunk_out, uint8_t *const *d_cls_out, uint8_t *const *d_flags,
-                       hipStream_t stream);
 void launch_seg_summary(SegDev *d_segs, int n_segs, const int32_t *d_first_seg, int n_chunks, int64_t *idx_base, uint32_t *seq_base, uint32_t *rec_off,
                         uint32_t *aux_off, ChunkSummary *d_out, hipStream_t stream);
-void launch_seg_gather(const SegDev *d_segs, int n_segs, const int64_t *idx_base, const uint32_t *seq_base, const uint32_t *rec_off,
-                       const uint32_t *aux_off, FixRec *out_recs, uint8_t *out_aux, hipStream_t stream);
+void launch_seg_finish(const SegDev *d_segs, int n_segs, const SegPiece *d_work, int n_work, uint8_t *const *d_chunk_out, uint8_t *const *d_cls_out,
+                       uint8_t *const *d_flags, const int64_t *idx_base, const uint32_t *seq_base, const uint32_t *rec_off, const uint32_t *aux_off,
+                       const ChunkSummary *d_sum, FixRec *out_recs, uint8_t *out_aux, hipStream_t stream);
 
 }
diff --git a/jasper_amd/csrc/polish_host.hip b/jasper_amd/csrc/polish_host.hip
--- a/jasper_amd/csrc/polish_host.hip
+++ b/jasper_amd/csrc/polish_host.hip
@@ -82,20 +82,25 @@
     DevBuf b_textA, b_textB, b_pack, b_cls, b_clsB, b_flags, b_segedit, b_cells, b_arrive, b_ptrA, b_segs, b_segtext, b_segrec, b_segaux, b_pool, b_locks, b_scan, b_ticket;
     DevBuf b_first, b_sum, b_idx, b_seq, b_ro, b_ao;
     DevBuf b_iooffs;
-    static constexpr size_t PIN_RECS = 1u << 18, PIN_AUX = 8u << 20;
+    static constexpr size_t PIN_OUT = (size_t)(1u << 18) * sizeof(FixRec) + (8u << 20);
+    uint8_t *table_p = nullptr;
+    size_t first_bytes = 0;
     SegDev *segs_p = nullptr;
     int32_t *first_p = nullptr;
+    SegDev *d_segs = nullptr;
+    SegPiece *d_work = nullptr;
+    size_t n_work = 0;
+    std::vector<SegPiece> work_h;
     ChunkSummary *sum_p = nullptr;
     int64_t *cand_p = nullptr;
-    FixRec *recs_p = nullptr;
-    uint8_t *aux_p = nullptr;
+    uint8_t *out_p = nullptr;
     ScanChunk *sc_p = nullptr;
     uint8_t *io_stage = nullptr;
     bool packed_io = false;
     int64_t total_len = 0;
     std::vector<int64_t> io_offs;
-    size_t pin_recs_used = 0, pin_aux_used = 0;
-    struct PinnedPass { size_t rec_at, nrec, aux_at, naux, r0, pass_i; };
+    size_t pin_out_used = 0;
+    struct PinnedPass { size_t at, nrec, naux, r0, pass_i; };
     std::vector<PinnedPass> pinned_passes;
 
     std::vector<uint8_t *> tables;
@@ -154,8 +159,7 @@
             STEP(host_bookkeeping(segs, n_chunks, pass, passes, books, pc, R, err));
         }
         STEP(account_chunks(len.data(), L, pc, pass, passes, R, err));
-        STEP(gather());
-        return stitch_and_swap();
+        return finish_pass();
     }
 
     bool ws(DevBuf &b, size_t bytes) {
@@ -194,12 +198,14 @@
     }
 
     int allocate() {
+        first_bytes = al256(((size_t)n_chunks + 1) * 4);
+        const size_t table_bytes = first_bytes + (size_t)L.max_segs * sizeof(SegDev) + max_pieces((size_t)L.max_segs, L.text_bytes) * sizeof(SegPiece);
         if (!ws(b_textA, L.text_bytes) || !ws(b_textB, L.text_bytes) ||
             !ws(b_cls, L.pos_items) || !ws(b_clsB, L.pos_items) || !ws(b_flags, L.flag_items) ||
             !ws(b_segedit, L.seg_rec_bound * sizeof(EditRec)) || !ws(b_cells, (2 + L.cell_items + L.cand_items) * 8) ||
             !ws(b_arrive, ((size_t)L.max_segs + 4) * 8) ||
             !ws(b_ptrA, (size_t)6 * n_chunks * sizeof(void *)) ||
-            !ws(b_segs, (size_t)L.max_segs * sizeof(SegDev)) || !ws(b_segtext, L.seg_text_bound) ||
+            !ws(b_segs, table_bytes) || !ws(b_segtext, L.seg_text_bound) ||
             !ws(b_segrec, L.seg_rec_bound * sizeof(FixRec)) || !ws(b_segaux, L.seg_aux_bound))
             return -2;
         pool.nslots = 256;
@@ -215,14 +221,15 @@
             !ws(b_ticket, 256)) return -2;
         if (!ws(b_first, ((size_t)n_chunks + 1) * 4) || !ws(b_sum, (size_t)n_chunks * sizeof(ChunkSummary)) || !ws(b_idx, (size_t)L.max_segs * 8) ||
             !ws(b_seq, (size_t)L.max_segs * 4) || !ws(b_ro, (size_t)L.max_segs * 4) || !ws(b_ao, (size_t)L.max_segs * 4)) return -2;
-        segs_p = pin<SegDev>(0, (size_t)L.max_segs * sizeof(SegDev));
-        first_p = pin<int32_t>(1, ((size_t)n_chunks + 1) * 4);
+        table_p = pin<uint8_t>(0, table_bytes);
         sum_p = pin<ChunkSummary>(2, (size_t)n_chunks * sizeof(ChunkSummary));
         cand_p = pin<int64_t>(3, (std::min<size_t>(L.cand_items, 32768) + L.cell_items + 8) * 8);
-        recs_p = pin<FixRec>(4, PIN_RECS * sizeof(FixRec));
-        aux_p = pin<uint8_t>(5, PIN_AUX);
+        out_p = pin<uint8_t>(4, PIN_OUT);
         sc_p = pin<ScanChunk>(6, sizeof(ScanChunk) * (size_t)n_chunks);
-        if (!segs_p || !first_p || !sum_p || !cand_p || !recs_p || !aux_p || !sc_p) return -2;
+        if (!table_p || !sum_p || !cand_p || !out_p || !sc_p) return -2;
+        first_p = reinterpret_cast<int32_t *>(table_p);
+        segs_p = reinterpret_cast<SegDev *>(table_p + first_bytes);
+        d_segs = reinterpret_cast<SegDev *>(b_segs.as<uint8_t>() + first_bytes);
         for (int c = 0; c < n_chunks; ++c) total_len += len[c];
         packed_io = !device_in && n_chunks > 256 && total_len / n_chunks < 65536 && !opt.no_packed_io;
         if (!packed_io) ws_next += 2;
@@ -255,6 +262,7 @@
 
     int upload() {
         HIPCHK(hipMemsetAsync(pool.locks, 0, pool.nslots * 4, st));
+        HIPCHK(hipMemsetAsync(d_count, 0, 4, st));
         clsIn = b_cls.as<uint8_t>();
         clsOut = b_clsB.as<uint8_t>();
         tables.resize((size_t)6 * n_chunks);
@@ -293,7 +301,6 @@
     }
 
     int scan() {
-        HIPCHK(hipMemsetAsync(d_count, 0, 4, st));
         for (int c = 0; c < n_chunks; ++c) {
             ScanChunk &S = sc[c];
             S.text = hIn[c];
@@ -347,24 +354,33 @@
         if (!nsv) return 0;
         const bool fine = opt.debug && opt.debug_level >= 2;
         double tf[5] = {fine ? now_ms() : 0, 0, 0, 0, 0};
-        if (hipMemcpyAsync(b_segs.p, sv, nsv * sizeof(SegDev), hipMemcpyHostToDevice, st) != hipSuccess) { err = "polish: H2D segs"; return -1; }
-        if (summary && hipMemcpyAsync(b_first.p, first_p, ((size_t)n_chunks + 1) * 4, hipMemcpyHostToDevice, st) != hipSuccess) { err = "polish: H2D first"; return -1; }
+        d_work = reinterpret_cast<SegPiece *>(d_segs + nsv);
+        if (sv == segs_p) {
+            n_work = make_pieces(sv, nsv, reinterpret_cast<SegPiece *>(sv + nsv));
+            if (hipMemcpyAsync(b_segs.p, table_p, first_bytes + nsv * sizeof(SegDev) + n_work * sizeof(SegPiece), hipMemcpyHostToDevice, st) != hipSuccess) { err = "polish: H2D segs"; return -1; }
+        } else {
+            work_h.resize(max_pieces(nsv, L.text_bytes));
+            n_work = make_pieces(sv, nsv, work_h.data());
+            if (hipMemcpyAsync(d_segs, sv, nsv * sizeof(SegDev), hipMemcpyHostToDevice, st) != hipSuccess) { err = "polish: H2D segs"; return -1; }
+            if (hipMemcpyAsync(d_work, work_h.data(), n_work * sizeof(SegPiece), hipMemcpyHostToDevice, st) != hipSuccess) { err = "polish: H2D pieces"; return -1; }
+        }
         if (fine) { (void)jk_stream_wait(st); tf[1] = now_ms(); }
-        launch_seg_init(b_segs.as<SegDev>(), (int)nsv, (const uint8_t *const *)dIn, st);
-        if (hipMemsetAsync(b_arrive.p, 0x80, (nsv + 2) * 8, st) != hipSuccess) { err = "polish: memset"; return -1; }
+        const PassPreset preset{b_arrive.as<long long>(), (int64_t)nsv + 2, b_ticket.as<unsigned int>(), reinterpret_cast<unsigned int *>(d_count),
+                                b_flags.as<uint8_t>(), (int64_t)(L.flag_items / 16)};
+        launch_seg_init(d_segs, d_work, (int)n_work, (const uint8_t *const *)dIn, preset, st);
         if (fine) { (void)jk_stream_wait(st); tf[2] = now_ms(); }
-        launch_seg_walk(T.d, b_segs.as<SegDev>(), (int)nsv, pp, pass, pool, b_ticket.as<unsigned int>(), st);
+        launch_seg_walk(T.d, d_segs, (int)nsv, pp, pass, pool, b_ticket.as<unsigned int>(), st);
         if (hipGetLastError() != hipSuccess) { err = "polish: kernel launch failed"; return -1; }
         if (fine) { (void)jk_stream_wait(st); tf[3] = now_ms(); }
         if (summary) {
-            launch_seg_summary(b_segs.as<SegDev>(), (int)nsv, b_first.as<int32_t>(), n_chunks, b_idx.as<int64_t>(), b_seq.as<uint32_t>(), b_ro.as<uint32_t>(),
+            launch_seg_summary(d_segs, (int)nsv, b_segs.as<int32_t>(), n_chunks, b_idx.as<int64_t>(), b_seq.as<uint32_t>(), b_ro.as<uint32_t>(),
                                b_ao.as<uint32_t>(), b_sum.as<ChunkSummary>(), st);
             if (hipMemcpyAsync(sum_p, b_sum.p, (size_t)n_chunks * sizeof(ChunkSummary), hipMemcpyDeviceToHost, st) != hipSuccess) { err = "polish: D2H summary"; return -1; }
-        } else if (hipMemcpyAsync(sv, b_segs.p, nsv * sizeof(SegDev), hipMemcpyDeviceToHost, st) != hipSuccess) { err = "polish: D2H segs"; return -1; }
+        } else if (hipMemcpyAsync(sv, d_segs, nsv * sizeof(SegDev), hipMemcpyDeviceToHost, st) != hipSuccess) { err = "polish: D2H segs"; return -1; }
         if (jk_stream_wait(st) != hipSuccess) { err = "polish: kernel execution failed"; return -1; }
         if (fine) {
             tf[4] = now_ms();
-            fprintf(stderr, "[polish]     %zu segments x %zu B: H2D %.3f ms, init + memset %.3f ms, walk %.3f ms, %s %.3f ms\n", nsv, sizeof(SegDev), tf[1] - tf[0], tf[2] - tf[1],
+            fprintf(stderr, "[polish]     %zu segments x %zu B: H2D %.3f ms, init %.3f ms, walk %.3f ms, %s %.3f ms\n", nsv, sizeof(SegDev), tf[1] - tf[0], tf[2] - tf[1],
                     tf[3] - tf[2], summary ? "summary + D2H" : "D2H", tf[4] - tf[3]);
         }
         return 0;
@@ -372,7 +388,7 @@
 
     int fetch_table() {
         segs.resize(ns);
-        HIPCHK(hipMemcpyAsync(segs.data(), b_segs.p, ns * sizeof(SegDev), hipMemcpyDeviceToHost, st));
+        HIPCHK(hipMemcpyAsync(segs.data(), d_segs, ns * sizeof(SegDev), hipMemcpyDeviceToHost, st));
         HIPCHK(jk_stream_wait(st));
         R.n_segments += segs.size();
         return 0;
@@ -427,47 +443,46 @@
         fprintf(stderr, "[polish]   segments by walk time: <0.1ms %d, <0.3 %d, <1 %d, <2 %d, <4 %d, <8 %d, <16 %d, more %d\n", hb[0], hb[1], hb[2], hb[3], hb[4], hb[5], hb[6], hb[7]);
     }
 
-    int gather() {
+    int finish_pass() {
         rec_pass_begin.push_back(R.recs.size());
         aux_pass.emplace_back();
         if (!ordinary) {
-            HIPCHK(hipMemcpyAsync(b_segs.p, segs.data(), ns * sizeof(SegDev), hipMemcpyHostToDevice, st));
+            work_h.resize(max_pieces(ns, L.text_bytes));
+            n_work = make_pieces(segs.data(), ns, work_h.data());
+            d_work = reinterpret_cast<SegPiece *>(d_segs + ns);
+            HIPCHK(hipMemcpyAsync(d_segs, segs.data(), ns * sizeof(SegDev), hipMemcpyHostToDevice, st));
+            HIPCHK(hipMemcpyAsync(d_work, work_h.data(), n_work * sizeof(SegPiece), hipMemcpyHostToDevice, st));
             HIPCHK(hipMemcpyAsync(b_idx.p, books.idx_base.data(), ns * 8, hipMemcpyHostToDevice, st));
             HIPCHK(hipMemcpyAsync(b_seq.p, books.seq_base.data(), ns * 4, hipMemcpyHostToDevice, st));
             HIPCHK(hipMemcpyAsync(b_ro.p, books.rec_off.data(), ns * 4, hipMemcpyHostToDevice, st));
             HIPCHK(hipMemcpyAsync(b_ao.p, books.aux_off.data(), ns * 4, hipMemcpyHostToDevice, st));
         }
-        if (!pc.nrec) return 0;
-        DevBuf d_recs, d_aux;
-        const int ws_save = ws_next;
-        if (!ws(d_recs, pc.nrec * sizeof(FixRec)) || !ws(d_aux, pc.naux)) return -2;
-        ws_next = ws_save;
-        launch_seg_gather(b_segs.as<SegDev>(), (int)ns, b_idx.as<int64_t>(), b_seq.as<uint32_t>(), b_ro.as<uint32_t>(), b_ao.as<uint32_t>(), d_recs.as<FixRec>(),
-                          d_aux.as<uint8_t>(), st);
+        DevBuf d_out;
+        const size_t rec_bytes = pc.nrec * sizeof(FixRec), out_bytes = rec_bytes + pc.naux;
+        if (pc.nrec) {
+            const int ws_save = ws_next;
+            if (!ws(d_out, out_bytes)) return -2;
+            ws_next = ws_save;
+        }
+        const bool carry = pass < passes;
+        launch_seg_finish(d_segs, (int)ns, d_work, (int)n_work, (uint8_t *const *)dOut, carry ? (uint8_t *const *)ptrClsOut : nullptr,
+                          carry ? (uint8_t *const *)ptrFlags : nullptr, b_idx.as<int64_t>(), b_seq.as<uint32_t>(), b_ro.as<uint32_t>(), b_ao.as<uint32_t>(),
+                          ordinary ? b_sum.as<ChunkSummary>() : nullptr, d_out.as<FixRec>(), d_out.as<uint8_t>() + rec_bytes, st);
         HIPCHK(hipGetLastError());
-        const size_t r0 = R.recs.size();
-        R.recs.resize(r0 + pc.nrec);
-        aux_pass.back().resize(pc.naux);
-        if (pin_recs_used + pc.nrec <= PIN_RECS && pin_aux_used + pc.naux <= PIN_AUX) {
-            HIPCHK(hipMemcpyAsync(recs_p + pin_recs_used, d_recs.p, pc.nrec * sizeof(FixRec), hipMemcpyDeviceToHost, st));
-            if (pc.naux) HIPCHK(hipMemcpyAsync(aux_p + pin_aux_used, d_aux.p, pc.naux, hipMemcpyDeviceToHost, st));
-            pinned_passes.push_back(PinnedPass{pin_recs_used, pc.nrec, pin_aux_used, pc.naux, r0, aux_pass.size() - 1});
-            pin_recs_used += pc.nrec;
-            pin_aux_used += pc.naux;
-        } else {
-            HIPCHK(hipMemcpyAsync(&R.recs[r0], d_recs.p, pc.nrec * sizeof(FixRec), hipMemcpyDeviceToHost, st));
-            if (pc.naux) HIPCHK(hipMemcpyAsync(aux_pass.back().data(), d_aux.p, pc.naux, hipMemcpyDeviceToHost, st));
-            HIPCHK(jk_stream_wait(st));
-        }
-        return 0;
-    }
-
-    int stitch_and_swap() {
-        const bool carry = pass < passes;
-        if (carry) HIPCHK(hipMemsetAsync(b_flags.p, 0, L.flag_items, st));
-        launch_seg_stitch(b_segs.as<SegDev>(), (int)ns, (uint8_t *const *)dOut, carry ? (uint8_t *const *)ptrClsOut : nullptr,
-                          carry ? (uint8_t *const *)ptrFlags : nullptr, st);
-        HIPCHK(hipGetLastError());
+        if (pc.nrec) {
+            const size_t r0 = R.recs.size();
+            R.recs.resize(r0 + pc.nrec);
+            aux_pass.back().resize(pc.naux);
+            if (pin_out_used + out_bytes <= PIN_OUT) {
+                HIPCHK(hipMemcpyAsync(out_p + pin_out_used, d_out.p, out_bytes, hipMemcpyDeviceToHost, st));
+                pinned_passes.push_back(PinnedPass{pin_out_used, pc.nrec, pc.naux, r0, aux_pass.size() - 1});
+                pin_out_used += (out_bytes + 31) & ~(size_t)31;
+            } else {
+                HIPCHK(hipMemcpyAsync(&R.recs[r0], d_out.p, rec_bytes, hipMemcpyDeviceToHost, st));
+                if (pc.naux) HIPCHK(hipMemcpyAsync(aux_pass.back().data(), d_out.as<uint8_t>() + rec_bytes, pc.naux, hipMemcpyDeviceToHost, st));
+                HIPCHK(jk_stream_wait(st));
+            }
+        }
         for (int c = 0; c < n_chunks; ++c) len[c] = pc.newlen[c];
         if (!ordinary) HIPCHK(jk_stream_wait(st));
         std::swap(hIn, hOut);
@@ -509,8 +524,8 @@
         HIPCHK(hipEventElapsedTime(&ms, ev0.e, ev1.e));
         R.seconds = ms * 1e-3;
         for (const PinnedPass &P : pinned_passes) {
-            memcpy(&R.recs[P.r0], recs_p + P.rec_at, P.nrec * sizeof(FixRec));
-            if (P.naux) memcpy(aux_pass[P.pass_i].data(), aux_p + P.aux_at, P.naux);
+            memcpy(&R.recs[P.r0], out_p + P.at, P.nrec * sizeof(FixRec));
+            if (P.naux) memcpy(aux_pass[P.pass_i].data(), out_p + P.at + P.nrec * sizeof(FixRec), P.naux);
         }
         regroup_and_sort(R, rec_pass_begin, aux_pass);
         return 0;
```

Measured after the change: 3109 (median of 6 runs). 1.01x the previous value.
